# dbekaert/RAiDER

Hardware: AMD Instinct MI355X
Metric: LOS rays/sec (wet+hydro slant delay) through ERA5 cube; achieved HBM GB/s (higher is better)
Workload: dtype f64; 1 GPU; configs[2]: Raytracing LOS, 4000x4000 scene (16.0M rays), one slice at ht=0, per-pixel ECEF look vectors, synthetic ERA5-sized 300x300x80 f32 cube, zref=max(z)-1, MAX_SEGMENT_LENGTH=1000; rays_per_gpu=16000000, cube=300x300x80, levels_K=76, parallelism=single GPU, ranks=1, world_size_seen_by_backend=1, devices_visible=1, ranks_per_device=1, distinct_devices=1

## Files before the change

### include/raider_hip.h

```cpp
#ifndef RAIDER_HIP_H
#define RAIDER_HIP_H

#include <stdint.h>

#ifdef __cplusplus
extern "C" {
#endif

#define RDR_OK 0
#define RDR_ERR_INVALID (-1)
#define RDR_ERR_HIP (-2)
#define RDR_ERR_NODEVICE (-3)
#define RDR_ERR_ALL_NAN (-4)
#define RDR_ERR_NO_LEVELS (-5)
#define RDR_ERR_NAN_LENGTH (-6)
#define RDR_ERR_OOM (-7)

#define RDR_F32 0
#define RDR_F64 1
#define RDR_I16 2
#define RDR_BYTESWAPPED 0x100
#define RDR_HOST 0
#define RDR_DEVICE 1

// ... 57 lines not shown
int rdr_clock_sample_end(rdr_ctx* ctx, double* ghz);
int rdr_ray_kernel_attributes(rdr_ctx* ctx, const rdr_cube* cube, int which, int32_t* vgprs, int32_t* static_lds, int32_t* dynamic_lds,
                              int32_t* scratch, int32_t* max_threads);
int64_t rdr_generic_ray_count(rdr_ctx* ctx);
int64_t rdr_skipped_wave_count(rdr_ctx* ctx);

int rdr_cube_create(rdr_ctx* ctx, const double* ys, int64_t ny, const double* xs, int64_t nx,
                    const double* zs, int64_t nz, const void* wet, const void* hydro, int dtype,
                    int64_t sy, int64_t sx, int64_t sz, int loc, rdr_cube** out);
void rdr_cube_destroy(rdr_cube* cube);
int rdr_cube_has_nan(const rdr_cube* cube);
int rdr_cube_shape(const rdr_cube* cube, int64_t* ny, int64_t* nx, int64_t* nz, int* dtype);
int rdr_cube_axes(const rdr_cube* cube, double* ys, double* xs, double* zs);
#define RDR_PROJ_LONLAT 0
#define RDR_PROJ_LCC 1
#define RDR_PROJ_STERE 2
int rdr_cube_set_projection(rdr_cube* cube, int kind, const double* params, int nparams);
int rdr_cube_view(rdr_ctx* ctx, const rdr_cube* cube, int kind, const double* params, int nparams, rdr_cube** out);
int rdr_project_points(rdr_ctx* ctx, const rdr_cube* cube, const double* lat, const double* lon, int64_t n, double* y, double* x, int loc);
int rdr_transform_tm(rdr_ctx* ctx, const double* params, int nparams, int direction, const double* in_a, const double* in_b, int64_t n,
                     double* out_a, double* out_b, int loc);
int rdr_transform_cone(rdr_ctx* ctx, int kind, const double* params, int nparams, int direction, const double* in_a, const double* in_b,
                       int64_t n, double* out_a, double* out_b, int loc);
#define RDR_GRID_TM 3
int rdr_grid_geodetic(rdr_ctx* ctx, int grid_kind, const double* params, int nparams, const double* xpts, int64_t nx, const double* ypts,
                      int64_t ny, double* lat, double* lon, int loc);
int rdr_cube_blend(rdr_ctx* ctx, const rdr_cube* a, double w1, const rdr_cube* b, double w2, rdr_cube** out);
int rdr_inverse_time_weights(rdr_ctx* ctx, const double* az, int64_t n, const double* dates, int32_t nd, double window_s,
                             double regularizer, double* weights, int loc);
int rdr_cube_blend_weighted(rdr_ctx* ctx, const rdr_cube* const* cubes, int32_t nd, const double* weights, int loc, rdr_cube** out);
int rdr_cube_blend_azimuth_time(rdr_ctx* ctx, const rdr_cube* const* pointwise, const rdr_cube* const* total, int32_t nd, const double* lat2d,
                                const double* lon2d, int loc, const double* sv_t, const double* sv_pos, const double* sv_vel, int64_t nsv,
                                const double* dates_s, double window_s, double reg, int64_t offset_us, rdr_cube** out_pointwise,
                                rdr_cube** out_total, double* time_grid, int32_t* flags);

int rdr_delays_to_phase(rdr_ctx* ctx, const void* wet, const void* hydro, int64_t n, int dtype, double wavelength,
                        void* wet_out, void* hydro_out, int loc);

int rdr_cube_read(rdr_ctx* ctx, const rdr_cube* cube, void* wet, void* hydro);

int rdr_interp3(rdr_ctx* ctx, const rdr_cube* cube, const double* pts, int64_t n, double* wet,
                double* hydro, int loc);
int rdr_interp3_project(rdr_ctx* ctx, const rdr_cube* cube, const double* y, const double* x, const double* z, int64_t n, int proj_mode,
                        const double* proj, double inc0, double* wet, double* hydro, int loc);
int rdr_cube_point_index(rdr_ctx* ctx, rdr_cube* cube, int mode);
int64_t rdr_cube_point_index_bytes(const rdr_cube* cube);
int rdr_build_cube(rdr_ctx* ctx, const rdr_cube* cube, const double* xpts, int64_t nx, const double* ypts,
                   int64_t ny, const double* zpts, int64_t nz, double* wet, double* hydro, int loc);
int rdr_build_cube_grid(rdr_ctx* ctx, const rdr_cube* cube, int grid_kind, const double* params, int nparams, const double* xpts, int64_t nx,
                        const double* ypts, int64_t ny, const double* zpts, int64_t nz, double* wet, double* hydro, int loc);
int rdr_last_nan_output(rdr_ctx* ctx);
int rdr_build_cube_to_cube(rdr_ctx* ctx, const rdr_cube* cube, const double* xpts, int64_t nx, const double* ypts, int64_t ny,
                           const double* zpts, int64_t nz, int loc, rdr_cube** out);
int rdr_build_cube_grid_to_cube(rdr_ctx* ctx, const rdr_cube* cube, int grid_kind, const double* params, int nparams, const double* xpts,
                                int64_t nx, const double* ypts, int64_t ny, const double* zpts, int64_t nz, int loc, rdr_cube** out);
int rdr_interp3_blend(rdr_ctx* ctx, const rdr_cube* a, double w1, const rdr_cube* b, double w2, const double* y, const double* x, const double* z,
                      int64_t n, double* wet, double* hydro, int loc);
int rdr_interp3_blend_cube(rdr_ctx* ctx, const rdr_cube* a, double w1, const rdr_cube* b, double w2, const double* y, const double* x, const double* z,
                           int64_t n, double* wet, double* hydro, int loc);
int rdr_point_delays(rdr_ctx* ctx, const rdr_cube* cube, const double* xpts, int64_t nx, const double* ypts, int64_t ny, const double* zpts,
                     int64_t nz, const double* y, const double* x, const double* z, int64_t n, int proj_mode, const double* proj, double inc0,
                     double* wet, double* hydro, int32_t* cube_has_nan);
int rdr_point_delays_grid(rdr_ctx* ctx, const rdr_cube* cube, int grid_kind, const double* params, int nparams, const double* xpts, int64_t nx,
                          const double* ypts, int64_t ny, const double* zpts, int64_t nz, const double* y, const double* x, const double* z, int64_t n,
                          int proj_mode, const double* proj, double inc0, double* wet, double* hydro, int32_t* cube_has_nan);
int rdr_interp3_project_epochs(rdr_ctx* ctx, const rdr_cube* const* cubes, int32_t ncubes, const double* y, const double* x, const double* z,
                               int64_t n, int proj_mode, const double* proj, int64_t proj_stride, double inc0, double* wet, double* hydro, int loc);
int rdr_point_delays_epochs(rdr_ctx* ctx, const rdr_cube* const* cubes, int32_t ncubes, int grid_kind, const double* params, int nparams,
                            const double* xpts, int64_t nx, const double* ypts, int64_t ny, const double* zpts, int64_t nz, const double* y,
                            const double* x, const double* z, int64_t n, int proj_mode, const double* proj, int64_t proj_stride, double inc0,
                            double* wet, double* hydro, int32_t* cube_has_nan);
int64_t rdr_point_upload_bytes(const rdr_ctx* ctx);
int rdr_project_cosinc(rdr_ctx* ctx, double* wet, double* hydro, const double* inc, int64_t n, int loc);
int rdr_project_divide(rdr_ctx* ctx, double* wet, double* hydro, const double* divisor, int64_t n, int loc);

int rdr_ray_levels(const rdr_cube* cube, double ht, double zref, int32_t* K, double* lo, double* hi, int32_t* kz);
int rdr_ray_prepass(rdr_ctx* ctx, const rdr_cube* cube, const rdr_rays* rays, double ht, double zref,
                    double* maxlen, int32_t* flags);
int rdr_nparts(const double* maxlen, int32_t K, double max_seg, int32_t* nparts);
int rdr_ray_prepass_device(rdr_ctx* ctx, const rdr_cube* cube, const rdr_rays* rays, double ht, double zref, double* partition);
int rdr_ray_march_device(rdr_ctx* ctx, const rdr_cube* cube, const rdr_rays* rays, double ht, double zref, double max_seg,
                         const double* partition, double* wet, double* hydro);

int rdr_ray_march(rdr_ctx* ctx, const rdr_cube* cube, const rdr_rays* rays, double ht, double zref,
                  const int32_t* nparts, int32_t flags, double* wet, double* hydro);
int rdr_raytrace(rdr_ctx* ctx, const rdr_cube* cube, const rdr_rays* rays, double ht, double zref,
                 double max_seg, double* wet, double* hydro, int32_t* nparts_out, int32_t* flags_out);

int rdr_raytrace_slices(rdr_ctx* ctx, const rdr_cube* cube, const rdr_rays* rays, const double* hts, int32_t nslices,
                        int32_t los_per_slice, double zref, double max_seg, double* wet, double* hydro, int32_t* K_out,
                        int32_t* nparts_out, int32_t ld, int32_t* flags_out);

int rdr_raytrace_slices_to_cube(rdr_ctx* ctx, const rdr_cube* cube, const rdr_rays* rays, const double* hts, int32_t nslices,
                                int32_t los_per_slice, double zref, double max_seg, int32_t* K_out, int32_t* nparts_out, int32_t ld,
                                int32_t* flags_out, rdr_cube** out);

int rdr_raytrace_slices_epochs(rdr_ctx* ctx, const rdr_cube* const* cubes, int32_t ncubes, const rdr_rays* rays, const double* hts,
                               int32_t nslices, int32_t los_per_slice, double zref, double max_seg, double* wet, double* hydro,
                               int32_t* K_out, int32_t* nparts_out, int32_t ld, int32_t* flags_out);

int rdr_raytrace_slices_epochs_to_cubes(rdr_ctx* ctx, const rdr_cube* const* cubes, int32_t ncubes, const rdr_rays* rays,
                                        const double* hts, int32_t nslices, int32_t los_per_slice, double zref, double max_seg,
                                        int32_t* K_out, int32_t* nparts_out, int32_t ld, int32_t* flags_out, rdr_cube** out);

int rdr_raytrace_epochs(rdr_ctx* ctx, const rdr_cube* const* cubes, int32_t ncubes, const rdr_rays* rays, double ht, double zref,
                        double max_seg, double* wet, double* hydro, int32_t* nparts_out, int32_t* flags_out);

int rdr_top_of_atmosphere(rdr_ctx* ctx, const double* xyz, const double* los, int64_t n, double toaheight,
                          const double* factor, double* pos, int loc);
int rdr_build_ray(rdr_ctx* ctx, const double* model_zs, int64_t nz, double ht, const double* xyz,
                  const double* los, int64_t n, double zref, int32_t* K, double* lengths, double* low,
                  double* high, int loc);

int rdr_lla2ecef(rdr_ctx* ctx, const double* lat, const double* lon, const double* h, int64_t n, double* xyz, int loc);
int rdr_ecef2lla(rdr_ctx* ctx, const double* xyz, int64_t n, double* lon, double* lat, double* h, int loc);
int rdr_look_vectors(rdr_ctx* ctx, const rdr_rays* rays, double ht, double* los);

int rdr_ecmwf_model_levels(rdr_ctx* ctx, const float* z_surf, const float* lnsp, const float* t, const float* q, const float* lats,
                           const double* a, const double* b, int32_t nlev, int64_t ny, int64_t nx, double R_d,
                           double* p_out, double* zs_out, int loc);

int rdr_pressure_level_state(rdr_ctx* ctx, const double* height, int height_kind, const double* p, int p_ndim, const double* t,
                             const double* hum, const double* lats, int lat_ndim, int64_t nlev, int64_t ny, int64_t nx,
                             int top_first, int rows_descending, int cols_descending, double* zs_out, double* p_out,
                             double* t_out, double* hum_out, int loc, int out_loc);

int rdr_cubes_from_model_levels(rdr_ctx* ctx, const double* ys, int64_t ny, const double* xs, int64_t nx, const double* zs3,
                                const double* p, const double* t, const double* hum, int humidity_type, int64_t nlev,
                                const double* new_z, int64_t nz, double k1, double k2, double k3, double zmin, int loc,
                                rdr_cube** pointwise, rdr_cube** total, float* t_out, float* p_out, float* e_out);

int rdr_orbit_look_vectors(rdr_ctx* ctx, const double* sv_t, const double* sv_pos, const double* sv_vel, int64_t nsv,
                           const double* xyz, int64_t n, double threshold, int maxiter, double* los, double* aztime,
                           double* srange, int loc);

int rdr_interp_nd(rdr_ctx* ctx, int32_t ndim, const double* const* axes, const int64_t* axis_len,
                  const double* values, const double* interp_points, int64_t n, int has_fill,
                  double fill_value, double* out, int loc);
int rdr_interp_along_axis(rdr_ctx* ctx, const double* points, const double* values, int64_t ncol, int64_t m,
                          const double* interp_points, int64_t mq, int has_fill, double fill_value,
                          double* out, int loc);
int64_t rdr_make_points_count(double max_len, double step);
int rdr_make_points(rdr_ctx* ctx, double max_len, const double* sp, const double* slv, int64_t nrays,
                    double step, double* out, int loc);

int rdr_raster_sample(rdr_ctx* ctx, const void* raster, int dtype, int64_t height, int64_t width, const double* gt6, const double* x,
                      const double* y, int64_t n, int method, int has_nodata, double nodata, double* out, int loc);
int rdr_raster_bounds(rdr_ctx* ctx, const void* a, const void* b, int dtype, int64_t n, int has_nodata, double nodata, double* out6, int loc);

int rdr_tiff_lzw_decode(rdr_ctx* ctx, const void* src, int64_t src_bytes, const int64_t* seg_offset, const int64_t* seg_bytes, int64_t nseg,
                        const int64_t* seg_out_bytes, void* out, int64_t out_stride, int32_t* status, int loc);
int rdr_tiff_assemble(rdr_ctx* ctx, const void* segs, int64_t seg_stride, int64_t height, int64_t width, int64_t tile_h, int64_t tile_w,
                      int predictor, int swap, int sample_bytes, int planar, int bands, int band, void* out, int loc);
int rdr_tiff_predict(rdr_ctx* ctx, const void* in, int sample_bytes, int64_t height, int64_t width, void* out, int loc);

int64_t rdr_deflate_bound(int64_t n);
int rdr_deflate_encode(rdr_ctx* ctx, const void* src, int64_t src_bytes, const int64_t* seg_offset, const int64_t* seg_bytes, int64_t nseg,
                       void* out, int64_t out_capacity, int64_t* out_offset, int loc);
int rdr_h5_chunks(rdr_ctx* ctx, const void* array, int elem_bytes, int ndim, const int64_t* shape, const int64_t* chunk, const void* fill,
                  int shuffle, void* out, int loc);

#ifdef __cplusplus
}
#endif
#endif
```

### raider_amd/_lib.py

```python
import ctypes as C
import os
import threading
from pathlib import Path

import numpy as np

_HERE = Path(__file__).resolve().parent
LIB_PATH = Path(os.environ.get('RAIDER_HIP_LIB', _HERE / 'libraider_hip.so'))

RDR_OK = 0
RDR_ERR_INVALID, RDR_ERR_HIP, RDR_ERR_NODEVICE, RDR_ERR_ALL_NAN, RDR_ERR_NO_LEVELS, RDR_ERR_NAN_LENGTH, RDR_ERR_OOM = -1, -2, -3, -4, -5, -6, -7
RDR_F32, RDR_F64, RDR_I16 = 0, 1, 2
RASTER_NEAREST, RASTER_LINEAR = 0, 1
RDR_BYTESWAPPED = 0x100
RDR_HOST, RDR_DEVICE = 0, 1
ORIGIN_GRID, ORIGIN_LLH, ORIGIN_XYZ = 0, 1, 2
RDR_PROJ_LCC, RDR_PROJ_STERE, RDR_GRID_TM = 1, 2, 3
LOS_VEC, LOS_INC_HD, LOS_INC_HD_SCALAR, LOS_ZENITH = 0, 1, 2, 3
ORBIT_LDS_MAX_SV = 320
FLAG_ANY_NAN, FLAG_ANY_FINITE, FLAG_FIRST_NOT_BELOW, FLAG_LAST_NOT_ABOVE, FLAG_DIVERGED, FLAG_BAD_HEIGHT, FLAG_NAN_OUTPUT = 1, 2, 4, 8, 16, 32, 64

c_dp = C.POINTER(C.c_double)
c_ip = C.POINTER(C.c_int32)
c_lp = C.POINTER(C.c_int64)
# ... 19 lines not shown


_lib = None
_lock = threading.Lock()

_VP = C.c_void_p
SYMBOLS = [
    ('rdr_version', C.c_int, []),
    ('rdr_source_hash', C.c_char_p, []),
    ('rdr_create', C.c_int, [C.c_int, C.POINTER(_VP)]),
    ('rdr_destroy', None, [_VP]),
    ('rdr_last_error', C.c_char_p, [_VP]),
    ('rdr_set_stream', C.c_int, [_VP, _VP]),
    ('rdr_forget_stream', C.c_int, [_VP, _VP]),
    ('rdr_synchronize', C.c_int, [_VP]),
    ('rdr_device_info', C.c_int, [_VP, C.c_char_p, C.c_int, C.POINTER(C.c_int), c_lp]),
    ('rdr_set_profiling', C.c_int, [_VP, C.c_int]),
    ('rdr_host_alloc', C.c_int, [C.c_int64, C.POINTER(_VP)]),
    ('rdr_host_free', C.c_int, [_VP]),
    ('rdr_set_workspace_limit', C.c_int, [_VP, C.c_int64]),
    ('rdr_set_side_capacity', C.c_int, [_VP, C.c_int64]),
    ('rdr_trim', C.c_int, [_VP, C.c_int64, c_lp]),
    ('rdr_generic_ray_count', C.c_int64, [_VP]),
    ('rdr_skipped_wave_count', C.c_int64, [_VP]),
    ('rdr_profile_get', C.c_int, [_VP, C.c_int, C.POINTER(C.c_int), C.POINTER(C.c_float)]),
    ('rdr_clock_sample_begin', C.c_int, [_VP, C.c_double]),
    ('rdr_clock_sample_end', C.c_int, [_VP, c_dp]),
    ('rdr_ray_kernel_attributes', C.c_int, [_VP, _VP, C.c_int, c_ip, c_ip, c_ip, c_ip, c_ip]),
    ('rdr_cube_create', C.c_int, [_VP, _VP, C.c_int64, _VP, C.c_int64, _VP, C.c_int64, _VP, _VP, C.c_int,
                                  C.c_int64, C.c_int64, C.c_int64, C.c_int, C.POINTER(_VP)]),
    ('rdr_cube_destroy', None, [_VP]),
    ('rdr_cube_has_nan', C.c_int, [_VP]),
    ('rdr_cube_shape', C.c_int, [_VP, c_lp, c_lp, c_lp, C.POINTER(C.c_int)]),
    ('rdr_cube_axes', C.c_int, [_VP, _VP, _VP, _VP]),
    ('rdr_cube_set_projection', C.c_int, [_VP, C.c_int, _VP, C.c_int]),
    ('rdr_cube_view', C.c_int, [_VP, _VP, C.c_int, _VP, C.c_int, C.POINTER(_VP)]),
    ('rdr_project_points', C.c_int, [_VP, _VP, _VP, _VP, C.c_int64, _VP, _VP, C.c_int]),
    ('rdr_transform_tm', C.c_int, [_VP, _VP, C.c_int, C.c_int, _VP, _VP, C.c_int64, _VP, _VP, C.c_int]),
    ('rdr_transform_cone', C.c_int, [_VP, C.c_int, _VP, C.c_int, C.c_int, _VP, _VP, C.c_int64, _VP, _VP, C.c_int]),
    ('rdr_grid_geodetic', C.c_int, [_VP, C.c_int, _VP, C.c_int, _VP, C.c_int64, _VP, C.c_int64, _VP, _VP, C.c_int]),
    ('rdr_cube_blend', C.c_int, [_VP, _VP, C.c_double, _VP, C.c_double, C.POINTER(_VP)]),
    ('rdr_cube_read', C.c_int, [_VP, _VP, _VP, _VP]),
    ('rdr_cube_point_index', C.c_int, [_VP, _VP, C.c_int]),
    ('rdr_cube_point_index_bytes', C.c_int64, [_VP]),
    ('rdr_interp3', C.c_int, [_VP, _VP, _VP, C.c_int64, _VP, _VP, C.c_int]),
    ('rdr_interp3_project', C.c_int, [_VP, _VP, _VP, _VP, _VP, C.c_int64, C.c_int, _VP, C.c_double, _VP, _VP, C.c_int]),
    ('rdr_interp3_blend', C.c_int, [_VP, _VP, C.c_double, _VP, C.c_double, _VP, _VP, _VP, C.c_int64, _VP, _VP, C.c_int]),
    ('rdr_interp3_blend_cube', C.c_int, [_VP, _VP, C.c_double, _VP, C.c_double, _VP, _VP, _VP, C.c_int64, _VP, _VP, C.c_int]),
    ('rdr_build_cube', C.c_int, [_VP, _VP, _VP, C.c_int64, _VP, C.c_int64, _VP, C.c_int64, _VP, _VP, C.c_int]),
    ('rdr_build_cube_to_cube', C.c_int, [_VP, _VP, _VP, C.c_int64, _VP, C.c_int64, _VP, C.c_int64, C.c_int, C.POINTER(_VP)]),
    ('rdr_build_cube_grid', C.c_int, [_VP, _VP, C.c_int, _VP, C.c_int, _VP, C.c_int64, _VP, C.c_int64, _VP, C.c_int64, _VP, _VP, C.c_int]),
    ('rdr_build_cube_grid_to_cube', C.c_int, [_VP, _VP, C.c_int, _VP, C.c_int, _VP, C.c_int64, _VP, C.c_int64, _VP, C.c_int64, C.c_int, C.POINTER(_VP)]),
    ('rdr_last_nan_output', C.c_int, [_VP]),
    ('rdr_point_delays', C.c_int, [_VP, _VP, _VP, C.c_int64, _VP, C.c_int64, _VP, C.c_int64, _VP, _VP, _VP, C.c_int64, C.c_int, _VP, C.c_double, _VP, _VP,
                                   c_ip]),
    ('rdr_point_delays_grid', C.c_int, [_VP, _VP, C.c_int, _VP, C.c_int, _VP, C.c_int64, _VP, C.c_int64, _VP, C.c_int64, _VP, _VP, _VP, C.c_int64, C.c_int,
                                        _VP, C.c_double, _VP, _VP, c_ip]),
    ('rdr_interp3_project_epochs', C.c_int, [_VP, C.POINTER(_VP), C.c_int32, _VP, _VP, _VP, C.c_int64, C.c_int, _VP, C.c_int64, C.c_double, _VP, _VP, C.c_int]),
    ('rdr_point_delays_epochs', C.c_int, [_VP, C.POINTER(_VP), C.c_int32, C.c_int, _VP, C.c_int, _VP, C.c_int64, _VP, C.c_int64, _VP, C.c_int64, _VP, _VP, _VP,
                                          C.c_int64, C.c_int, _VP, C.c_int64, C.c_double, _VP, _VP, c_ip]),
    ('rdr_point_upload_bytes', C.c_int64, [_VP]),
    ('rdr_project_cosinc', C.c_int, [_VP, _VP, _VP, _VP, C.c_int64, C.c_int]),
    ('rdr_project_divide', C.c_int, [_VP, _VP, _VP, _VP, C.c_int64, C.c_int]),
    ('rdr_ray_levels', C.c_int, [_VP, C.c_double, C.c_double, c_ip, _VP, _VP, _VP]),
    ('rdr_ray_prepass', C.c_int, [_VP, _VP, C.POINTER(RdrRays), C.c_double, C.c_double, _VP, c_ip]),
    ('rdr_nparts', C.c_int, [_VP, C.c_int32, C.c_double, _VP]),
    ('rdr_ray_march', C.c_int, [_VP, _VP, C.POINTER(RdrRays), C.c_double, C.c_double, _VP, C.c_int32, _VP, _VP]),
    ('rdr_raytrace', C.c_int, [_VP, _VP, C.POINTER(RdrRays), C.c_double, C.c_double, C.c_double, _VP, _VP, _VP, c_ip]),
    ('rdr_raytrace_slices', C.c_int, [_VP, _VP, C.POINTER(RdrRays), _VP, C.c_int32, C.c_int32, C.c_double, C.c_double, _VP, _VP, _VP, _VP, C.c_int32, _VP]),
    ('rdr_raytrace_slices_to_cube', C.c_int, [_VP, _VP, C.POINTER(RdrRays), _VP, C.c_int32, C.c_int32, C.c_double, C.c_double, _VP, _VP, C.c_int32, _VP,
                                              C.POINTER(_VP)]),
    ('rdr_raytrace_slices_epochs', C.c_int, [_VP, C.POINTER(_VP), C.c_int32, C.POINTER(RdrRays), _VP, C.c_int32, C.c_int32, C.c_double, C.c_double,
                                             _VP, _VP, _VP, _VP, C.c_int32, _VP]),
    ('rdr_raytrace_slices_epochs_to_cubes', C.c_int, [_VP, C.POINTER(_VP), C.c_int32, C.POINTER(RdrRays), _VP, C.c_int32, C.c_int32, C.c_double,
                                                      C.c_double, _VP, _VP, C.c_int32, _VP, C.POINTER(_VP)]),
    ('rdr_raytrace_epochs', C.c_int, [_VP, C.POINTER(_VP), C.c_int32, C.POINTER(RdrRays), C.c_double, C.c_double, C.c_double, _VP, _VP, _VP, c_ip]),
    ('rdr_top_of_atmosphere', C.c_int, [_VP, _VP, _VP, C.c_int64, C.c_double, _VP, _VP, C.c_int]),
    ('rdr_build_ray', C.c_int, [_VP, _VP, C.c_int64, C.c_double, _VP, _VP, C.c_int64, C.c_double, c_ip, _VP, _VP, _VP, C.c_int]),
    ('rdr_lla2ecef', C.c_int, [_VP, _VP, _VP, _VP, C.c_int64, _VP, C.c_int]),
    ('rdr_ecef2lla', C.c_int, [_VP, _VP, C.c_int64, _VP, _VP, _VP, C.c_int]),
    ('rdr_look_vectors', C.c_int, [_VP, C.POINTER(RdrRays), C.c_double, _VP]),
    ('rdr_ray_prepass_device', C.c_int, [_VP, _VP, _VP, C.c_double, C.c_double, _VP]),
    ('rdr_ray_march_device', C.c_int, [_VP, _VP, _VP, C.c_double, C.c_double, C.c_double, _VP, _VP, _VP]),
    ('rdr_inverse_time_weights', C.c_int, [_VP, _VP, C.c_int64, _VP, C.c_int32, C.c_double, C.c_double, _VP, C.c_int]),
    ('rdr_cube_blend_weighted', C.c_int, [_VP, C.POINTER(_VP), C.c_int32, _VP, C.c_int, C.POINTER(_VP)]),
    ('rdr_cube_blend_azimuth_time', C.c_int, [_VP, C.POINTER(_VP), C.POINTER(_VP), C.c_int32, _VP, _VP, C.c_int, _VP, _VP, _VP, C.c_int64, _VP, C.c_double,
                                              C.c_double, C.c_int64, C.POINTER(_VP), C.POINTER(_VP), _VP, c_ip]),
    ('rdr_delays_to_phase', C.c_int, [_VP, _VP, _VP, C.c_int64, C.c_int, C.c_double, _VP, _VP, C.c_int]),
    ('rdr_ecmwf_model_levels', C.c_int, [_VP, _VP, _VP, _VP, _VP, _VP, _VP, _VP, C.c_int32, C.c_int64, C.c_int64, C.c_double, _VP, _VP, C.c_int]),
    ('rdr_pressure_level_state', C.c_int, [_VP, _VP, C.c_int, _VP, C.c_int, _VP, _VP, _VP, C.c_int, C.c_int64, C.c_int64, C.c_int64, C.c_int, C.c_int,
                                           C.c_int, _VP, _VP, _VP, _VP, C.c_int, C.c_int]),
    ('rdr_cubes_from_model_levels', C.c_int, [_VP, _VP, C.c_int64, _VP, C.c_int64, _VP, _VP, _VP, _VP, C.c_int, C.c_int64, _VP, C.c_int64,
                                              C.c_double, C.c_double, C.c_double, C.c_double, C.c_int, C.POINTER(_VP), C.POINTER(_VP), _VP, _VP, _VP]),
    ('rdr_orbit_look_vectors', C.c_int, [_VP, _VP, _VP, _VP, C.c_int64, _VP, C.c_int64, C.c_double, C.c_int, _VP, _VP, _VP, C.c_int]),
    ('rdr_interp_nd', C.c_int, [_VP, C.c_int32, C.POINTER(_VP), c_lp, _VP, _VP, C.c_int64, C.c_int, C.c_double, _VP, C.c_int]),
    ('rdr_interp_along_axis', C.c_int, [_VP, _VP, _VP, C.c_int64, C.c_int64, _VP, C.c_int64, C.c_int, C.c_double, _VP, C.c_int]),
    ('rdr_make_points_count', C.c_int64, [C.c_double, C.c_double]),
    ('rdr_make_points', C.c_int, [_VP, C.c_double, _VP, _VP, C.c_int64, C.c_double, _VP, C.c_int]),
    ('rdr_raster_sample', C.c_int, [_VP, _VP, C.c_int, C.c_int64, C.c_int64, _VP, _VP, _VP, C.c_int64, C.c_int, C.c_int, C.c_double, _VP, C.c_int]),
    ('rdr_raster_bounds', C.c_int, [_VP, _VP, _VP, C.c_int, C.c_int64, C.c_int, C.c_double, _VP, C.c_int]),
    ('rdr_tiff_lzw_decode', C.c_int, [_VP, _VP, C.c_int64, _VP, _VP, C.c_int64, _VP, _VP, C.c_int64, _VP, C.c_int]),
    ('rdr_tiff_assemble', C.c_int, [_VP, _VP, C.c_int64, C.c_int64, C.c_int64, C.c_int64, C.c_int64, C.c_int, C.c_int, C.c_int, C.c_int, C.c_int, C.c_int,
                                    _VP, C.c_int]),
    ('rdr_tiff_predict', C.c_int, [_VP, _VP, C.c_int, C.c_int64, C.c_int64, _VP, C.c_int]),
    ('rdr_deflate_bound', C.c_int64, [C.c_int64]),
    ('rdr_deflate_encode', C.c_int, [_VP, _VP, C.c_int64, _VP, _VP, C.c_int64, _VP, C.c_int64, _VP, C.c_int]),
    ('rdr_h5_chunks', C.c_int, [_VP, _VP, C.c_int, C.c_int, _VP, _VP, _VP, C.c_int, _VP, C.c_int]),
]


def _preload_hip_runtime():
    import importlib.util
    import sys
    choice = os.environ.get('RAIDER_HIP_RUNTIME', '')
    if choice == 'system' or 'torch' in sys.modules:
        return
    if choice:
        C.CDLL(choice, mode=C.RTLD_GLOBAL)
        return
    try:
        spec = importlib.util.find_spec('torch')
    except (ImportError, ValueError):
        spec = None
    if spec and spec.submodule_search_locations:
        cand = Path(list(spec.submodule_search_locations)[0]) / 'lib' / 'libamdhip64.so'
        if cand.exists():
            C.CDLL(str(cand), mode=C.RTLD_GLOBAL)


def source_files():
    return sorted(f for f in (_HERE / 'csrc').glob('*') if f.suffix in ('.h', '.hip')) + [_HERE.parent / 'include' / 'raider_hip.h']


def source_hash():
    import hashlib
    h = hashlib.sha256()
    for f in source_files():
        h.update(f.name.encode()); h.update(f.read_bytes())
    return h.hexdigest()[:16]


def binary_source_hash(path=None):
    path = Path(path or LIB_PATH)
    if not path.exists():
        return None
    if _lib is not None and path == LIB_PATH:
        return _lib.rdr_source_hash().decode()
    data = path.read_bytes()
    k = data.find(b'rdr-source-hash:')
    if k < 0:
        return None
    return data[k + 16:k + 32].decode(errors='replace')


def load():
    global _lib
    with _lock:
        if _lib is not None:
            return _lib
        if not LIB_PATH.exists():
            raise RuntimeError(
                f'raider_amd: HIP library {LIB_PATH} is missing - build it with '
                f'`python -c "import __graft_entry__ as g; g.build()"` (hipcc --offload-arch=gfx950). '
                'There is no CPU fallback.')
        _preload_hip_runtime()
        lib = C.CDLL(str(LIB_PATH))
# ... 157 lines not shown
```

### raider_amd/csrc/epoch_kernels.h

```cpp
#pragma once
#include "raider_kernels.h"
#include "cube_kernels.h"

namespace rdr {

constexpr int EPOCHS_MAX = 4;

template <typename T2, int E, bool PR>
struct EpochWaves {
    static constexpr int value = PR ? (sizeof(T2) == 8 ? (E <= 2 ? 3 : 2) : (E <= 2 ? 2 : 1)) : ((sizeof(T2) == 8 && E <= 2) ? 3 : 2);
};

template <typename T2, int E, int GRID, bool PR>
__global__ __launch_bounds__(BLOCK) __attribute__((amdgpu_waves_per_eu(EpochWaves<T2, E, PR>::value, EpochWaves<T2, E, PR>::value)))
void march_epochs_kernel(CubeView<T2> c_in, EpochCubes<T2, E> ev, RayParams P, int64_t estride) {
    static_assert(!PR || GRID == 0 || GRID == 1, "per-ray heights: REGULAR or run-time flags");
    constexpr bool REGULAR = GRID == 1;
    CubeView<T2> c = c_in;
    if (REGULAR) { c.exact_y = 1; c.exact_x = 1; c.small = 1; }
    if (GRID == 2) { c.exact_y = 0; c.exact_x = 0; c.uni_y = 1; c.uni_x = 1; c.small = 1; }
    extern __shared__ __attribute__((aligned(16))) unsigned char smem_raw[];
    const RaySmem m = carve_smem(smem_raw, c.ny, c.nx, c.nz, c.exact_y, c.exact_x);
    fill_axes(c, m);
    int K = 0, slice = -1;
    double poison = 0.0;
    bool clamp_lo = false, clamp_hi = false;
    TileWalk walk(P.tile_count, P.tile_ctr, m.K + 2);
    int64_t lt;
    while (walk.next(P.tile_count, lt)) {
        const int64_t tg = P.tile_begin + lt;
        const int sl = (int)(tg / P.tiles_per_slice);
        const int64_t t = tg - (int64_t)sl * P.tiles_per_slice;
        if (sl != slice) {
            slice = sl;
            K = fill_levels(c.nz, m, P.hts ? P.hts[sl] : P.ht, P.zref);
            const SlicePartition part = fill_partition<!PR>(P, m, c.nz, sl, K);
            poison = part.poison; clamp_lo = part.clamp_lo; clamp_hi = part.clamp_hi;
        }
        int tl = threadIdx.x;
        asm volatile("" : "+v"(tl));
        int64_t i; bool active;
        tile_ray(P, t, tl, i, active);
        const double* w = P.ws + (lt * BLOCK + tl);
        const int64_t ns = P.nslots;
        const double scale_rec = w[(int64_t)WS_SCALE * ns];
        const bool mine = !active || scale_rec != 0.0;
        int k0 = 0; double lo_first = K > 0 ? m.lo[0] : 0.0;
        if constexpr (PR) k0 = (active && mine) ? first_level(m.ax.ez, c.nz, m.lo, m.hi, m.kz, K, P.ht_ray[i], lo_first) : K;
        double acc_w[E], acc_h[E];
#pragma unroll
        for (int e = 0; e < E; ++e) { acc_w[e] = 0.0; acc_h[e] = 0.0; }
        RayPoly q;
        double xc[PX];
        load_ray_record(w, ns, q, xc);
        const double scale = scale_rec;
        const double u0r = w[(int64_t)WS_U0 * ns], u1r = w[(int64_t)WS_U1 * ns];
        const unsigned long long live = __builtin_amdgcn_ballot_w64(active && mine);
        auto run = [&](auto nochk) {
            constexpr bool NC = decltype(nochk)::value;
            if constexpr (PR) march_ray_height_levels<T2, E, NC>(c, ev, m, q, xc, u0r, u1r, K, k0, lo_first, clamp_lo, clamp_hi, acc_w, acc_h);
            else march_slice_levels<T2, E, NC>(c, ev, m, q, xc, u0r, u1r, K, clamp_lo, clamp_hi, live, acc_w, acc_h);
        };
        bool lane_safe = false;
        if (REGULAR) lane_safe = lane_nocheck(u0r, u1r, active, mine, q, xc, c.ny, c.nx);
        if (REGULAR && __all(lane_safe)) run(std::integral_constant<bool, true>{});
        else run(std::integral_constant<bool, false>{});
        if (active && scale_rec != 0.0) {
            const int64_t o = (int64_t)sl * P.n + i;
#pragma unroll
            for (int e = 0; e < E; ++e) {
                const double aw = acc_w[e] * scale, ah = acc_h[e] * scale;
                P.wet[e * estride + o] = aw + poison; P.hyd[e * estride + o] = ah + poison;
            }
        }
    }
}

template <typename T2, int E>
__global__ __launch_bounds__(256) void interp_points_epochs_kernel(CubeView<T2> c, EpochCubes<T2, E> ev, PointQuery Q, int64_t pstride, int64_t n, int64_t estride,
                                                                   double* __restrict__ wet, double* __restrict__ hyd, int axes_in_lds) {
    PlainCorners<T2> src[E];
#pragma unroll
    for (int e = 0; e < E; ++e) src[e].v = ev.v[e];
    gather_points<E>(c, src, Q, pstride, n, estride, wet, hyd, axes_in_lds);
}

}
```

### raider_amd/csrc/raider_hip.hip

```cpp
#include <hip/hip_runtime.h>

#include <algorithm>
#include <atomic>
#include <cmath>
#include <cstdio>
#include <cstdlib>
#include <cstring>
#include <functional>
#include <mutex>
#include <string>
#include <utility>
#include <vector>

#include "../../include/raider_hip.h"
#include "raider_kernels.h"

using namespace rdr;

static thread_local std::string g_err;

struct DevBuf {
    void* p = nullptr;
    size_t cap = 0;
};

constexpr int MAX_SLICES = 512;

enum { SLOT_IN0 = 0, SLOT_IN1, SLOT_IN2, SLOT_IN3, SLOT_IN4, SLOT_IN5, SLOT_IN6, SLOT_OUT0, SLOT_OUT1, SLOT_OUT2, SLOT_AUX,
       SLOT_PT0, SLOT_PT1, SLOT_PT2, SLOT_PT3, SLOT_PT4, SLOT_PT5, SLOT_TMPCUBE, SLOT_TMPAXES,
       SLOT_DEFL,
       NSLOT };

struct rdr_ctx {
    int device = 0;
    hipStream_t own_stream = nullptr;
    hipStream_t copy_stream = nullptr;
    hipStream_t down_stream = nullptr;
    hipStream_t stream = nullptr;
    int num_cus = 256;
    size_t lds_max = 64u << 10;
    size_t total_mem = 0;
    std::string name;
    bool profiling = false;
    std::vector<std::pair<hipEvent_t, hipEvent_t>> evs[4];
    size_t ev_used[4] = {0, 0, 0, 0};
    DevBuf slot[NSLOT];
    unsigned long long* d_maxlen = nullptr;
    int* d_flags = nullptr;
    int* d_nparts = nullptr;
    int* d_nslow = nullptr;
    int* d_tilectr = nullptr;
    struct PoolEntry { void* p; size_t bytes; std::vector<hipEvent_t> evs; };
    std::vector<PoolEntry> cube_pool;
    std::vector<hipStream_t> ext_streams;
    bool ext_overflow = false;
    size_t cube_pool_bytes = 0, cube_pool_limit = (size_t)4 << 30;
    DevBuf ws;
    DevBuf side;
    int64_t side_cap = 0;
    int* d_sidectr = nullptr;
    int* h_word = nullptr;
    struct PinSlot { void* p = nullptr; size_t cap = 0; hipEvent_t ev = nullptr; bool used = false; };
    static constexpr int PIN_SLOTS = 16;
    static constexpr size_t PIN_MAX = (size_t)1 << 20;
    PinSlot pin[PIN_SLOTS];
    int pin_next = 0;
    hipEvent_t staged_ev = nullptr;
    static constexpr int NAN_SLOTS = 256;
    int* nan_words = nullptr;
    const struct rdr_cube* nan_owner[NAN_SLOTS] = {};
    int nan_next = 0;
    int64_t side_forced = -1;
    int64_t last_nskip = 0;
    int64_t last_nslow = 0;
    int wall_khz = 0;
    int64_t point_upload_bytes = 0;
    int last_nan_output = -1;
    size_t ws_limit = (size_t)48 << 30;
    struct { const void* cube = nullptr; const void* vals = nullptr; LccParams proj = {0, 0, 0, 0, 0, 0, 0, 0}; int64_t n = -1; double ht = 0, zref = 0; const void* a = nullptr; const void* b = nullptr; const void* c = nullptr; const void* d = nullptr; int K = 0; bool valid = false; } wsig;
    std::string err;
};

struct rdr_cube {
    rdr_ctx* ctx = nullptr;
    int64_t ny = 0, nx = 0, nz = 0;
    int dtype = RDR_F32;
    void* d_vals = nullptr;
    double* d_axes = nullptr;
    std::vector<double> ys, xs, zs;
    int uni[3] = {0, 0, 0};
    int exact[2] = {0, 0};
    double inv_d[3] = {0, 0, 0};
    LccParams proj = {0, 0, 0, 0, 0, 0, 0, 0};
    mutable void* d_quad = nullptr;
    mutable size_t quad_bytes = 0;
    mutable int quad_nblk = 0;
    mutable int big_point_calls = 0;
    mutable std::mutex quad_mutex;
    mutable bool has_nan = false;
    mutable hipEvent_t ready_ev = nullptr;
    hipStream_t ready_stream = nullptr;
    mutable int nan_slot = -1;
    size_t alloc_bytes = 0;
    const rdr_cube* base = nullptr;
    mutable int views = 0;
    mutable bool doomed = false;
    mutable std::atomic<bool> foreign{false};
    mutable std::vector<hipStream_t> used_streams;
    mutable std::atomic<hipStream_t> last_stream{nullptr};
};
static std::recursive_mutex g_view_mutex;
static inline const rdr_cube* root(const rdr_cube* q) { return q->base ? q->base : q; }
static inline void note_use(const rdr_ctx* c, const rdr_cube* q) {
    if (!c || !q) return;
    const rdr_cube* r = root(q);
    if (r->ctx != c) r->foreign.store(true, std::memory_order_relaxed);
    if (r->last_stream.load(std::memory_order_relaxed) != c->stream) {
        std::lock_guard<std::recursive_mutex> guard(g_view_mutex);
        if (std::find(r->used_streams.begin(), r->used_streams.end(), c->stream) == r->used_streams.end()) r->used_streams.push_back(c->stream);
        r->last_stream.store(c->stream, std::memory_order_relaxed);
    }
    if (r->ready_ev && r->ready_stream != c->stream) { (void)hipStreamWaitEvent(c->stream, r->ready_ev, 0); (void)hipGetLastError(); }
}
static void cube_resolve_nan(const rdr_cube* r) {
    std::lock_guard<std::recursive_mutex> guard(g_view_mutex);
    if (r->nan_slot < 0) return;
    rdr_ctx* c = r->ctx;
    if (r->ready_ev) (void)hipEventSynchronize(r->ready_ev);
    r->has_nan = c->nan_words[r->nan_slot] != 0;
    c->nan_owner[r->nan_slot] = nullptr;
    r->nan_slot = -1;
}


static int fail(rdr_ctx* ctx, int code, const std::string& msg) {
    g_err = msg;
    if (ctx) ctx->err = msg;
    return code;
}

#define HIPCHECK(ctx, expr)                                                                         \
    do {                                                                                            \
// ... 144 lines not shown
    hipLaunchKernelGGL(kern, g, b, sm, s, std::forward<Args>(args)...);
    return hipGetLastError();
}

#include "cube_kernels.h"
#include "producer_kernels.h"
#include "orbit_kernels.h"
#include "aztime_kernels.h"
#include "native_kernels.h"
#include "proj_kernels.h"
#include "epoch_kernels.h"
#include "raster_kernels.h"
#include "tiff_kernels.h"
#include "deflate_kernels.h"


int rdr_version(void) { return 102; }

#ifndef RDR_SOURCE_HASH
#define RDR_SOURCE_HASH "unknown"
#endif
static const char k_source_hash[] = "rdr-source-hash:" RDR_SOURCE_HASH;
const char* rdr_source_hash(void) { return k_source_hash + 16; }

const char* rdr_last_error(rdr_ctx* ctx) { return (ctx && !ctx->err.empty()) ? ctx->err.c_str() : g_err.c_str(); }

int rdr_create(int device, rdr_ctx** out) {
    if (!out) return fail(nullptr, RDR_ERR_INVALID, "rdr_create: out is NULL");
    *out = nullptr;
    int count = 0;
    hipError_t e = hipGetDeviceCount(&count);
    if (e != hipSuccess || count <= 0)
        return fail(nullptr, RDR_ERR_NODEVICE, std::string("rdr_create: no HIP device available (") +
                    (e != hipSuccess ? hipGetErrorString(e) : "device count 0") + "); raider_amd has no CPU fallback");
    if (device < 0) { if (hipGetDevice(&device) != hipSuccess) device = 0; }
    if (device >= count) return fail(nullptr, RDR_ERR_INVALID, "rdr_create: device index out of range");
    rdr_ctx* c = new rdr_ctx();
    c->device = device;
    const int rc = [&]() -> int {
        HIPCHECK(nullptr, hipSetDevice(device));
        hipDeviceProp_t prop;
        HIPCHECK(nullptr, hipGetDeviceProperties(&prop, device));
        c->num_cus = prop.multiProcessorCount;
        c->total_mem = prop.totalGlobalMem;
        c->lds_max = std::max<size_t>(prop.sharedMemPerBlock, prop.maxSharedMemoryPerMultiProcessor);
        c->name = prop.name;
        if (c->name.empty()) c->name = std::string("AMD ") + prop.gcnArchName;
        HIPCHECK(nullptr, hipStreamCreateWithFlags(&c->own_stream, hipStreamNonBlocking));
        HIPCHECK(nullptr, hipStreamCreateWithFlags(&c->copy_stream, hipStreamNonBlocking));
        HIPCHECK(nullptr, hipStreamCreateWithFlags(&c->down_stream, hipStreamNonBlocking));
        c->stream = c->own_stream;
        HIPCHECK(nullptr, hipMalloc((void**)&c->d_maxlen, (size_t)MAX_SLICES * MAX_LEVELS * sizeof(unsigned long long)));
        HIPCHECK(nullptr, hipMalloc((void**)&c->d_flags, (MAX_SLICES + 4) * sizeof(int)));
        HIPCHECK(nullptr, hipMalloc((void**)&c->d_nparts, MAX_LEVELS * sizeof(int)));
        HIPCHECK(nullptr, hipMalloc((void**)&c->d_nslow, 2 * sizeof(int)));
        HIPCHECK(nullptr, hipMalloc((void**)&c->d_tilectr, 32 * sizeof(int)));
        HIPCHECK(nullptr, hipMalloc((void**)&c->d_sidectr, sizeof(int)));
        HIPCHECK(nullptr, hipMemset(c->d_sidectr, 0, sizeof(int)));
        HIPCHECK(nullptr, hipHostMalloc((void**)&c->h_word, 16 * sizeof(int), hipHostMallocDefault));
        HIPCHECK(nullptr, hipHostMalloc((void**)&c->nan_words, rdr_ctx::NAN_SLOTS * sizeof(int), hipHostMallocDefault));
        HIPCHECK(nullptr, hipMemset(c->d_nslow, 0, 2 * sizeof(int)));
        return RDR_OK;
    }();
    if (rc) { rdr_destroy(c); return rc; }
    if (const char* e = std::getenv("RAIDER_HIP_WORKSPACE_BYTES")) c->ws_limit = (size_t)std::strtoull(e, nullptr, 10);
    if (const char* e = std::getenv("RAIDER_HIP_CUBE_POOL_BYTES")) c->cube_pool_limit = (size_t)std::strtoull(e, nullptr, 10);
    *out = c;
    return RDR_OK;
}

void rdr_destroy(rdr_ctx* c) {
    if (!c) return;
    (void)hipSetDevice(c->device);
    if (c->stream) (void)hipStreamSynchronize(c->stream);
    for (auto& b : c->slot) if (b.p) (void)hipFree(b.p);
    for (auto& e : c->cube_pool) { for (auto ev : e.evs) (void)hipEventDestroy(ev); (void)hipFree(e.p); }
    if (c->d_maxlen) (void)hipFree(c->d_maxlen);
    if (c->d_flags) (void)hipFree(c->d_flags);
    if (c->d_nparts) (void)hipFree(c->d_nparts);
    if (c->d_nslow) (void)hipFree(c->d_nslow);
    if (c->d_tilectr) (void)hipFree(c->d_tilectr);
    if (c->ws.p) (void)hipFree(c->ws.p);
    if (c->side.p) (void)hipFree(c->side.p);
    if (c->d_sidectr) (void)hipFree(c->d_sidectr);
    if (c->h_word) (void)hipHostFree(c->h_word);
    if (c->nan_words) (void)hipHostFree(c->nan_words);
    for (auto& ps : c->pin) { if (ps.ev) (void)hipEventDestroy(ps.ev); if (ps.p) (void)hipHostFree(ps.p); }
    if (c->staged_ev) (void)hipEventDestroy(c->staged_ev);
    for (auto& v : c->evs) for (auto& pr : v) { (void)hipEventDestroy(pr.first); (void)hipEventDestroy(pr.second); }
    if (c->own_stream) (void)hipStreamDestroy(c->own_stream);
    if (c->copy_stream) (void)hipStreamDestroy(c->copy_stream);
    if (c->down_stream) (void)hipStreamDestroy(c->down_stream);
    delete c;
}

int rdr_set_stream(rdr_ctx* c, void* s) {
    if (!c) return fail(nullptr, RDR_ERR_INVALID, "ctx is NULL");
    const hipStream_t before = c->stream;
    const hipStream_t want = (s == (void*)(intptr_t)-1) ? c->own_stream : (hipStream_t)s;
    if (want != before) {
        hipEvent_t ev = nullptr;
        if (hipEventCreateWithFlags(&ev, hipEventDisableTiming) == hipSuccess) {
            if (hipEventRecord(ev, before) == hipSuccess) (void)hipStreamWaitEvent(want, ev, 0);
            (void)hipEventDestroy(ev);
        }
        (void)hipGetLastError();
    }
    if (s == (void*)(intptr_t)-1) c->stream = c->own_stream;
    else {
        c->stream = (hipStream_t)s;
        std::lock_guard<std::recursive_mutex> guard(g_view_mutex);
        if (std::find(c->ext_streams.begin(), c->ext_streams.end(), c->stream) == c->ext_streams.end()) {
            if (c->ext_streams.size() < 8) c->ext_streams.push_back(c->stream); else c->ext_overflow = true;
        }
    }
    return RDR_OK;
}

int rdr_forget_stream(rdr_ctx* c, void* s) {
    if (!c) return fail(nullptr, RDR_ERR_INVALID, "ctx is NULL");
    const hipStream_t st = (hipStream_t)s;
    if (c->stream == st && st != c->own_stream) {
        HIPCHECK(c, hipStreamSynchronize(st));
        c->stream = c->own_stream;
    }
    std::lock_guard<std::recursive_mutex> guard(g_view_mutex);
    c->ext_streams.erase(std::remove(c->ext_streams.begin(), c->ext_streams.end(), st), c->ext_streams.end());
    if (c->ext_streams.size() < 8) c->ext_overflow = false;
    return RDR_OK;
}

int rdr_synchronize(rdr_ctx* c) {
    if (!c) return fail(nullptr, RDR_ERR_INVALID, "ctx is NULL");
    HIPCHECK(c, hipStreamSynchronize(c->stream));
    return RDR_OK;
}

int rdr_device_info(rdr_ctx* c, char* name, int name_len, int* cus, int64_t* mem) {
    if (!c) return fail(nullptr, RDR_ERR_INVALID, "ctx is NULL");
    if (name && name_len > 0) { std::strncpy(name, c->name.c_str(), name_len - 1); name[name_len - 1] = 0; }
    if (cus) *cus = c->num_cus;
    if (mem) *mem = (int64_t)c->total_mem;
    return RDR_OK;
}

int rdr_host_alloc(int64_t bytes, void** out) {
    if (!out || bytes <= 0) return fail(nullptr, RDR_ERR_INVALID, "rdr_host_alloc: bad argument");
    void* p = nullptr;
    const hipError_t e = hipHostMalloc(&p, (size_t)bytes, hipHostMallocDefault);
    if (e != hipSuccess) return fail(nullptr, RDR_ERR_HIP, std::string("hipHostMalloc: ") + hipGetErrorString(e));
    *out = p;
    return RDR_OK;
}

int rdr_host_free(void* p) {
    if (!p) return RDR_OK;
    const hipError_t e = hipHostFree(p);
    if (e != hipSuccess) return fail(nullptr, RDR_ERR_HIP, std::string("hipHostFree: ") + hipGetErrorString(e));
    return RDR_OK;
}

int rdr_set_workspace_limit(rdr_ctx* c, int64_t bytes) {
    if (!c || bytes < (int64_t)1 << 20) return fail(c, RDR_ERR_INVALID, "rdr_set_workspace_limit: need at least 1 MiB");
    c->ws_limit = (size_t)bytes;
    c->wsig.valid = false;
    return RDR_OK;
}

static void pool_drain(rdr_ctx* c) {
    std::lock_guard<std::recursive_mutex> guard(g_view_mutex);
    while (!c->cube_pool.empty()) {
        rdr_ctx::PoolEntry e = c->cube_pool.front();
        c->cube_pool.erase(c->cube_pool.begin());
        c->cube_pool_bytes -= e.bytes;
        for (auto ev : e.evs) { (void)hipEventSynchronize(ev); (void)hipEventDestroy(ev); }
        (void)hipFree(e.p);
    }
    (void)hipGetLastError();
}

int rdr_trim(rdr_ctx* c, int64_t keep_bytes, int64_t* released) {
    if (!c || keep_bytes < 0) return fail(c, RDR_ERR_INVALID, "rdr_trim: NULL context or a negative size");
    HIPCHECK(c, hipSetDevice(c->device));
    HIPCHECK(c, hipStreamSynchronize(c->down_stream));
    HIPCHECK(c, hipStreamSynchronize(c->copy_stream));
    HIPCHECK(c, hipStreamSynchronize(c->stream));
    if (c->stream != c->own_stream) HIPCHECK(c, hipStreamSynchronize(c->own_stream));
    const size_t keep = (size_t)keep_bytes;
    size_t freed = 0;
    auto drop = [&](DevBuf& b) { if (b.p && b.cap > keep) { if (hipFree(b.p) == hipSuccess) freed += b.cap; b.p = nullptr; b.cap = 0; } };
    for (auto& b : c->slot) drop(b);
    if ((c->ws.p && c->ws.cap > keep) || (c->side.p && c->side.cap > keep)) c->wsig.valid = false;
    drop(c->ws);
    if (c->side.p && c->side.cap > keep) { drop(c->side); c->side_cap = 0; }
    std::lock_guard<std::recursive_mutex> guard(g_view_mutex);
    while (!c->cube_pool.empty() && c->cube_pool_bytes > keep) {
        rdr_ctx::PoolEntry e = c->cube_pool.front();
        c->cube_pool.erase(c->cube_pool.begin());
        c->cube_pool_bytes -= e.bytes;
        for (auto ev : e.evs) { (void)hipEventSynchronize(ev); (void)hipEventDestroy(ev); }
        if (hipFree(e.p) == hipSuccess) freed += e.bytes;
    }
    (void)hipGetLastError();
    if (released) *released = (int64_t)freed;
    return RDR_OK;
}

int rdr_set_side_capacity(rdr_ctx* c, int64_t columns) {
    if (!c) return fail(nullptr, RDR_ERR_INVALID, "ctx is NULL");
    c->side_forced = columns < 0 ? -1 : columns;
    c->wsig.valid = false;
    return RDR_OK;
}

int64_t rdr_generic_ray_count(rdr_ctx* c) { return c ? c->last_nslow : -1; }
int64_t rdr_skipped_wave_count(rdr_ctx* c) { return c ? c->last_nskip : -1; }

int rdr_set_profiling(rdr_ctx* c, int on) {
    if (!c) return fail(nullptr, RDR_ERR_INVALID, "ctx is NULL");
    c->profiling = on != 0;
    for (auto& u : c->ev_used) u = 0;
    return RDR_OK;
}

__global__ void clock_sample_kernel(long long wall_ticks, long long* out) {
    if (threadIdx.x != 0) return;
    const long long c0 = clock64(), w0 = wall_clock64();
    while (wall_clock64() - w0 < wall_ticks) __builtin_amdgcn_s_sleep(127);
    const long long c1 = clock64(), w1 = wall_clock64();
    out[0] = c1 - c0; out[1] = w1 - w0;
}

int rdr_clock_sample_begin(rdr_ctx* c, double ms) {
    if (!c || !(ms > 0) || ms > 60000.0) return fail(c, RDR_ERR_INVALID, "rdr_clock_sample_begin: NULL context or a duration outside (0, 60000] ms");
    HIPCHECK(c, hipSetDevice(c->device));
    int khz = 0;
    HIPCHECK(c, hipDeviceGetAttribute(&khz, hipDeviceAttributeWallClockRate, c->device));
    if (khz <= 0) return fail(c, RDR_ERR_HIP, "rdr_clock_sample_begin: the device reports no wall-clock rate");
    long long* out = reinterpret_cast<long long*>(c->h_word + 4);
    out[0] = 0; out[1] = 0;
    c->wall_khz = khz;
    hipLaunchKernelGGL(clock_sample_kernel, dim3(1), dim3(64), 0, c->copy_stream, (long long)(ms * khz), out);
    HIPCHECK(c, hipGetLastError());
    return RDR_OK;
}

int rdr_clock_sample_end(rdr_ctx* c, double* ghz) {
    if (!c || !ghz) return fail(c, RDR_ERR_INVALID, "rdr_clock_sample_end: NULL argument");
    HIPCHECK(c, hipSetDevice(c->device));
    HIPCHECK(c, hipStreamSynchronize(c->copy_stream));
    const long long* out = reinterpret_cast<const long long*>(c->h_word + 4);
    if (out[1] <= 0 || c->wall_khz <= 0) return fail(c, RDR_ERR_INVALID, "rdr_clock_sample_end: no sample was started on this context");
    *ghz = (double)out[0] / ((double)out[1] / (c->wall_khz * 1e3)) / 1e9;
    return RDR_OK;
}

int rdr_profile_get(rdr_ctx* c, int which, int* count, float* total_ms) {
    if (!c || which < 0 || which > 3 || !count || !total_ms) return fail(c, RDR_ERR_INVALID, "rdr_profile_get: bad argument");
    float tot = 0;
    for (size_t i = 0; i < c->ev_used[which]; ++i) {
        float ms = 0;
        HIPCHECK(c, hipEventSynchronize(c->evs[which][i].second));
        HIPCHECK(c, hipEventElapsedTime(&ms, c->evs[which][i].first, c->evs[which][i].second));
        tot += ms;
    }
    *count = (int)c->ev_used[which];
    *total_ms = tot;
    return RDR_OK;
}

static int axis_check(const double* g, int64_t n, int* flip) {
    if (n < 2) return -1;
    bool asc = true, desc = true;
    for (int64_t i = 1; i < n; ++i) {
        if (!(g[i] > g[i - 1])) asc = false;
        if (!(g[i] < g[i - 1])) desc = false;
    }
// ... 1259 lines not shown
    c->wsig.cube = q; c->wsig.vals = q->d_vals; c->wsig.proj = q->proj; c->wsig.n = r->n; c->wsig.ht = ht; c->wsig.zref = zref; c->wsig.K = K; c->wsig.valid = valid;
    c->wsig.a = r->origin_mode == RDR_ORIGIN_GRID ? (const void*)r->xpts : (r->origin_mode == RDR_ORIGIN_XYZ ? (const void*)r->xyz : (const void*)r->lat);
    c->wsig.b = r->origin_mode == RDR_ORIGIN_GRID ? (const void*)r->ypts : (const void*)r->lon;
    c->wsig.c = r->los_mode == RDR_LOS_VEC ? (const void*)r->los : (const void*)r->inc;
    c->wsig.d = (const void*)r->hts;
}

static bool wsig_match(rdr_ctx* c, const rdr_cube* q, const rdr_rays* r, double ht, double zref, int K) {
    if (!c->wsig.valid || c->wsig.cube != q || c->wsig.vals != q->d_vals || std::memcmp(&c->wsig.proj, &q->proj, sizeof(LccParams)) != 0 || c->wsig.n != r->n || c->wsig.ht != ht || c->wsig.zref != zref || c->wsig.K != K) return false;
    if (r->loc != RDR_DEVICE) return false;
    const void* a = r->origin_mode == RDR_ORIGIN_GRID ? (const void*)r->xpts : (r->origin_mode == RDR_ORIGIN_XYZ ? (const void*)r->xyz : (const void*)r->lat);
    const void* b = r->origin_mode == RDR_ORIGIN_GRID ? (const void*)r->ypts : (const void*)r->lon;
    const void* cc = r->los_mode == RDR_LOS_VEC ? (const void*)r->los : (const void*)r->inc;
    return a == c->wsig.a && b == c->wsig.b && cc == c->wsig.c && (const void*)r->hts == c->wsig.d;
}

static bool pass1_skip_on() {
    static const int on = []() { const char* e = std::getenv("RAIDER_HIP_PASS1_SKIP"); return e ? std::atoi(e) : 1; }();
    return on != 0;
}

template <typename T2>
static auto crossings_fn(bool lcc, int om, bool per_ray) -> void (*)(CubeView<T2>, RayParams, LccParams) {
#define RDR_X(LCC_, OM_) (per_ray ? crossings_kernel<T2, false, LCC_, OM_, true> : crossings_kernel<T2, false, LCC_, OM_, false>)
#define RDR_X_OM(LCC_) (om == 1 ? RDR_X(LCC_, 1) : om == 2 ? RDR_X(LCC_, 2) : RDR_X(LCC_, 0))
    return lcc ? RDR_X_OM(true) : RDR_X_OM(false);
#undef RDR_X_OM
#undef RDR_X
}

template <typename T2>
static auto march_fn(int grid, bool per_ray) -> void (*)(CubeView<T2>, RayParams, LccParams) {
    if (per_ray) return grid == 1 ? march_kernel<T2, false, 1, true> : march_kernel<T2, false, 0, true>;
    return grid == 1 ? march_kernel<T2, false, 1> : grid == 2 ? march_kernel<T2, false, 2> : march_kernel<T2, false, 0>;
}

template <typename T2, int E>
static auto march_epochs_fn(int grid, bool per_ray) -> void (*)(CubeView<T2>, EpochCubes<T2, E>, RayParams, int64_t) {
    if (per_ray) return grid == 1 ? march_epochs_kernel<T2, E, 1, true> : march_epochs_kernel<T2, E, 0, true>;
    return grid == 1 ? march_epochs_kernel<T2, E, 1, false> : grid == 2 ? march_epochs_kernel<T2, E, 2, false> : march_epochs_kernel<T2, E, 0, false>;
}

static int launch_crossings(rdr_ctx* c, const rdr_cube* q, RayParams P, int64_t tb, int64_t tc, int64_t nslots_total = 0, bool reset_nslow = true) {
    P.tile_begin = tb; P.tile_count = tc; P.nslots = nslots_total > 0 ? nslots_total : tc * BLOCK;
    const bool skippable = pass1_skip_on() && q->proj.kind != 1 && !P.ht_ray && P.maxlen_bits != nullptr &&
                           ray_lds_total(q) + skip_smem_bytes(q->nz) <= c->lds_max;
    P.skip_levels = skippable ? 1 : 0;
    const int g = ray_grid(c, tc, 8);
    if (ray_lds_total(q) > c->lds_max)
        return fail(c, RDR_ERR_INVALID, "ray tracing: the cube's non-uniform horizontal axes and level tables need " + std::to_string(ray_lds_total(q)) +
                    " B of LDS per workgroup, the device offers " + std::to_string(c->lds_max) + " (resample the cube to uniform axes or crop it)");
    if (reset_nslow) {
        HIPCHECK(c, hipMemsetAsync(c->d_nslow, 0, 2 * sizeof(int), c->stream));
        HIPCHECK(c, hipMemsetAsync(c->d_sidectr, 0, sizeof(int), c->stream));
    }
    HIPCHECK(c, hipMemsetAsync(c->d_tilectr, 0, 16 * sizeof(int), c->stream));
    P.tile_ctr = c->d_tilectr;
    const size_t sm = ray_smem(q);
    hipError_t e = hipSuccess;
    {
        KTimer t(c, 0);
        const size_t sm_light = sm + (skippable ? skip_smem_bytes(q->nz) : 0);
        const bool lcc = q->proj.kind == 1;
        const int om = P.origin_mode != RDR_ORIGIN_GRID ? 0 : (P.los_mode == RDR_LOS_VEC ? 1 : 2);
        const dim3 G(g), B(BLOCK);
        e = q->dtype == RDR_F32 ? launch_lds(crossings_fn<float2>(lcc, om, P.ht_ray != nullptr), G, B, sm_light, c->stream, make_view<float2>(q), P, q->proj)
                                : launch_lds(crossings_fn<double2>(lcc, om, P.ht_ray != nullptr), G, B, sm_light, c->stream, make_view<double2>(q), P, q->proj);
    }
    if (e != hipSuccess) return fail(c, RDR_ERR_HIP, std::string("crossings_kernel launch: ") + hipGetErrorString(e));
    P.tile_ctr = c->d_tilectr + 8;
    if (q->dtype == RDR_F32) e = launch_lds(crossings_kernel<float2, true>, dim3(g), dim3(BLOCK), sm, c->stream, make_view<float2>(q), P, q->proj);
    else e = launch_lds(crossings_kernel<double2, true>, dim3(g), dim3(BLOCK), sm, c->stream, make_view<double2>(q), P, q->proj);
    if (e != hipSuccess) return fail(c, RDR_ERR_HIP, std::string("crossings_kernel launch: ") + hipGetErrorString(e));
    return RDR_OK;
}

static int march_grid(const rdr_cube* q, bool per_ray) {
    const bool small = make_view<float2>(q).small && (q->dtype == RDR_F32 || make_view<double2>(q).small);
    if (!small) return 0;
    if (q->exact[0] && q->exact[1]) return 1;
    return (!per_ray && !q->exact[0] && !q->exact[1] && q->uni[0] && q->uni[1]) ? 2 : 0;
}

static int launch_march_generic(rdr_ctx* c, const rdr_cube* q, RayParams P, dim3 G, dim3 B, size_t sm, bool zero_ctr) {
    if (zero_ctr) HIPCHECK(c, hipMemsetAsync(c->d_tilectr + 24, 0, 8 * sizeof(int), c->stream));
    P.tile_ctr = c->d_tilectr + 24;
    hipError_t e;
    if (q->dtype == RDR_F32) e = launch_lds(march_kernel<float2, true>, G, B, sm, c->stream, make_view<float2>(q), P, q->proj);
    else e = launch_lds(march_kernel<double2, true>, G, B, sm, c->stream, make_view<double2>(q), P, q->proj);
    if (e != hipSuccess) return fail(c, RDR_ERR_HIP, std::string("march_kernel launch: ") + hipGetErrorString(e));
    return RDR_OK;
}

static int launch_march(rdr_ctx* c, const rdr_cube* q, RayParams P, int64_t tb, int64_t tc, int64_t nslots_total = 0) {
    P.tile_begin = tb; P.tile_count = tc; P.nslots = nslots_total > 0 ? nslots_total : tc * BLOCK;
    static const int stage_f64 = []() { const char* e = std::getenv("RAIDER_HIP_F64_STAGE"); return e ? std::atoi(e) : 1; }();
    P.stage_f64 = stage_f64;
    const int g = ray_grid(c, tc, 8);
    HIPCHECK(c, hipMemsetAsync(c->d_tilectr + 16, 0, 16 * sizeof(int), c->stream));
    P.tile_ctr = c->d_tilectr + 16;
    const size_t sm = ray_smem(q);
    const dim3 G(g), B(BLOCK);
    hipError_t e = hipSuccess;
    {
        KTimer t(c, 1);
        const bool per_ray = P.ht_ray != nullptr;
        const int grid = march_grid(q, per_ray);
        e = q->dtype == RDR_F32 ? launch_lds(march_fn<float2>(grid, per_ray), G, B, sm, c->stream, make_view<float2>(q), P, q->proj)
                                : launch_lds(march_fn<double2>(grid, per_ray), G, B, sm, c->stream, make_view<double2>(q), P, q->proj);
    }
    if (e != hipSuccess) return fail(c, RDR_ERR_HIP, std::string("march_kernel launch: ") + hipGetErrorString(e));
    return launch_march_generic(c, q, P, G, B, sm, false);
}

static int epochs_max() {
    const char* e = std::getenv("RAIDER_HIP_EPOCHS_MAX");
    const int v = e ? std::atoi(e) : EPOCHS_MAX;
    return v >= 4 ? 4 : v >= 2 ? 2 : 1;
}

static int epoch_group(int dtype, bool per_ray, int left, int emax) {
    if (per_ray && dtype == RDR_F64) {
        const char* env = std::getenv("RAIDER_HIP_EPOCHS_PR_F64_MAX");
        emax = std::min(emax, env ? std::atoi(env) : 2);
    }
    return (left >= 4 && emax >= 4) ? 4 : (left >= 2 && emax >= 2) ? 2 : 1;
}

template <typename T2, int E>
static hipError_t launch_stacked(rdr_ctx* c, const rdr_cube* const* qs, int grid, const RayParams& P, int64_t estride, dim3 G, dim3 B, size_t sm) {
    EpochCubes<T2, E> ev;
    for (int j = 0; j < E; ++j) ev.v[j] = (const T2*)qs[j]->d_vals;
    return launch_lds(march_epochs_fn<T2, E>(grid, P.ht_ray != nullptr), G, B, sm, c->stream, make_view<T2>(qs[0]), ev, P, estride);
}

static int launch_march_epochs(rdr_ctx* c, const rdr_cube* const* qs, int D, RayParams P, int64_t tb, int64_t tc, int64_t estride) {
    const rdr_cube* q = qs[0];
    const int emax = epochs_max();
    const bool per_ray = P.ht_ray != nullptr;
    const int grid = march_grid(q, per_ray);
    const int g = ray_grid(c, tc, 8);
    const size_t sm = ray_smem(q);
    const dim3 G(g), B(BLOCK);
    for (int e = 0; e < D;) {
        const int ge = epoch_group(q->dtype, per_ray, D - e, emax);
        RayParams Pe = P;
        Pe.wet = P.wet + (int64_t)e * estride; Pe.hyd = P.hyd + (int64_t)e * estride;
        if (ge == 1) {
            const int rc = launch_march(c, qs[e], Pe, tb, tc); if (rc) return rc;
            ++e;
            continue;
        }
        Pe.tile_begin = tb; Pe.tile_count = tc; Pe.nslots = tc * BLOCK;
        HIPCHECK(c, hipMemsetAsync(c->d_tilectr + 16, 0, 8 * sizeof(int), c->stream));
        Pe.tile_ctr = c->d_tilectr + 16;
        hipError_t err = hipSuccess;
        {
            KTimer t(c, 1);
            if (q->dtype == RDR_F32) err = ge == 4 ? launch_stacked<float2, 4>(c, qs + e, grid, Pe, estride, G, B, sm) : launch_stacked<float2, 2>(c, qs + e, grid, Pe, estride, G, B, sm);
            else err = ge == 4 ? launch_stacked<double2, 4>(c, qs + e, grid, Pe, estride, G, B, sm) : launch_stacked<double2, 2>(c, qs + e, grid, Pe, estride, G, B, sm);
        }
        if (err != hipSuccess) return fail(c, RDR_ERR_HIP, std::string("march_epochs_kernel launch: ") + hipGetErrorString(err));
        for (int j = 0; j < ge; ++j) {
            RayParams Pj = Pe;
            Pj.wet = Pe.wet + (int64_t)j * estride; Pj.hyd = Pe.hyd + (int64_t)j * estride;
            const int rc = launch_march_generic(c, qs[e + j], Pj, G, B, sm, true); if (rc) return rc;
        }
        e += ge;
    }
    return RDR_OK;
}

int rdr_ray_kernel_attributes(rdr_ctx* c, const rdr_cube* q, int which, int32_t* vgprs, int32_t* static_lds, int32_t* dynamic_lds,
                              int32_t* scratch, int32_t* max_threads) {
    if (!c || !q || which < 0 || which > 7) return fail(c, RDR_ERR_INVALID, "rdr_ray_kernel_attributes: bad argument");
    const void* fn = nullptr;
    const bool lcc = q->proj.kind == 1;
    const bool pr = which == 2 || which == 3 || which >= 6;
    const int grid = march_grid(q, pr);
    const bool f32 = q->dtype == RDR_F32;
    if (which >= 4) {
        if ((which & 1) != 0) fn = f32 ? (const void*)march_epochs_fn<float2, 4>(grid, pr) : (const void*)march_epochs_fn<double2, 4>(grid, pr);
        else fn = f32 ? (const void*)march_epochs_fn<float2, 2>(grid, pr) : (const void*)march_epochs_fn<double2, 2>(grid, pr);
    } else if ((which & 1) == 0) fn = f32 ? (const void*)crossings_fn<float2>(lcc, 1, pr) : (const void*)crossings_fn<double2>(lcc, 1, pr);
    else fn = f32 ? (const void*)march_fn<float2>(grid, pr) : (const void*)march_fn<double2>(grid, pr);
    hipFuncAttributes a;
    HIPCHECK(c, hipFuncGetAttributes(&a, fn));
    if (vgprs) *vgprs = a.numRegs;
    if (static_lds) *static_lds = (int32_t)a.sharedSizeBytes;
    if (dynamic_lds) *dynamic_lds = (int32_t)ray_smem(q);
    if (scratch) *scratch = (int32_t)a.localSizeBytes;
    if (max_threads) *max_threads = a.maxThreadsPerBlock;
    return RDR_OK;
}

static int ray_passes(rdr_ctx* c, const rdr_cube* q, const RayParams& P, int K, int64_t per, int64_t nslices, int64_t fit, int64_t max_group,
                      bool reduce, const std::function<int(const RayParams&, int64_t, int64_t)>& march = nullptr,
                      const std::function<int(int64_t, int64_t)>& after_group = nullptr) {
    const auto pass2 = [&](const RayParams& Pm, int64_t tb, int64_t tc) { return march ? march(Pm, tb, tc) : launch_march(c, q, Pm, tb, tc); };
    if (per <= fit) {
        const int64_t g = std::min<int64_t>(max_group, std::max<int64_t>(1, fit / per));
        for (int64_t s0 = 0; s0 < nslices; s0 += g) {
            const int64_t ns = std::min<int64_t>(g, nslices - s0);
            RayParams Pg = P;
            if (!reduce) Pg.maxlen_bits = nullptr;
            int rc = ws_reserve(c, ns * per, K, Pg); if (rc) return rc;
            rc = launch_crossings(c, q, Pg, s0 * per, ns * per); if (rc) return rc;
            Pg.maxlen_bits = P.maxlen_bits;
            rc = pass2(Pg, s0 * per, ns * per); if (rc) return rc;
            if (after_group) { rc = after_group(s0, ns); if (rc) return rc; }
        }
        return RDR_OK;
    }
    for (int64_t s = 0; s < nslices; ++s) {
        int rc;
        if (reduce) {
            RayParams Ps = P;
            Ps.ws = nullptr;
            rc = launch_crossings(c, q, Ps, s * per, per); if (rc) return rc;
        }
        RayParams Pw = P;
        rc = ws_reserve(c, fit, K, Pw); if (rc) return rc;
        for (int64_t tb = 0; tb < per; tb += fit) {
            const int64_t tc = std::min<int64_t>(fit, per - tb);
            RayParams Pc = Pw;
            Pc.maxlen_bits = nullptr;
            rc = launch_crossings(c, q, Pc, s * per + tb, tc); if (rc) return rc;
            Pc.maxlen_bits = P.maxlen_bits;
            rc = pass2(Pc, s * per + tb, tc); if (rc) return rc;
        }
    }
    return RDR_OK;
}

static int raytrace_pipelined(rdr_ctx* c, const rdr_cube* q, const rdr_rays* r, RayParams P, int K, double* d_los, double* d_hts, double* dw, double* dh,
                              double* wet, double* hydro) {
    const int64_t tile_rows = P.ntiles / P.tiles_x;
    const int nchunk = (int)std::min<int64_t>(8, tile_rows);
    int rc = ws_reserve(c, P.ntiles, K, P); if (rc) return rc;
    double* const ws = P.ws;
    const int64_t nslots_total = P.ntiles * BLOCK;
    if (d_los) P.los = d_los;
    if (d_hts) P.ht_ray = d_hts;
    std::vector<hipEvent_t> ev(2 * nchunk, nullptr);
    auto range = [&](int k, int64_t& tb, int64_t& tc, int64_t& r0, int64_t& cnt) {
        const int64_t t0 = tile_rows * k / nchunk, t1 = tile_rows * (k + 1) / nchunk;
        tb = t0 * P.tiles_x; tc = (t1 - t0) * P.tiles_x;
        if (r->origin_mode == RDR_ORIGIN_GRID) { r0 = t0 * TILE * r->nx; cnt = std::min<int64_t>(t1 * TILE, r->ny) * r->nx - r0; }
        else { r0 = tb * BLOCK; cnt = std::min<int64_t>((tb + tc) * BLOCK, r->n) - r0; }
    };
    int status = RDR_OK;
    auto cleanup = [&]() { for (auto& e : ev) if (e) (void)hipEventDestroy(e); };
    for (auto& e : ev)
        if (hipEventCreateWithFlags(&e, hipEventDisableTiming) != hipSuccess) { cleanup(); return fail(c, RDR_ERR_HIP, "pipelined ray tracing: event creation failed"); }
    for (int k = 0; k < nchunk && status == RDR_OK; ++k) {
        int64_t tb, tc, r0, cnt; range(k, tb, tc, r0, cnt);
        if ((d_los && hipMemcpyAsync(d_los + 3 * r0, r->los + 3 * r0, (size_t)cnt * 24, hipMemcpyHostToDevice, c->copy_stream) != hipSuccess) ||
            (d_hts && hipMemcpyAsync(d_hts + r0, r->hts + r0, (size_t)cnt * 8, hipMemcpyHostToDevice, c->copy_stream) != hipSuccess) ||
            ((d_los || d_hts) && (hipEventRecord(ev[k], c->copy_stream) != hipSuccess || hipStreamWaitEvent(c->stream, ev[k], 0) != hipSuccess))) {
            status = fail(c, RDR_ERR_HIP, "pipelined ray tracing: look-vector / height upload failed"); break;
        }
        RayParams Pk = P; Pk.ws = ws + tb * BLOCK;
        status = launch_crossings(c, q, Pk, tb, tc, nslots_total, k == 0);
    }
    for (int k = 0; k < nchunk && status == RDR_OK; ++k) {
        int64_t tb, tc, r0, cnt; range(k, tb, tc, r0, cnt);
        RayParams Pk = P; Pk.ws = ws + tb * BLOCK;
        status = launch_march(c, q, Pk, tb, tc, nslots_total);
        if (status == RDR_OK && hipEventRecord(ev[nchunk + k], c->stream) != hipSuccess) status = fail(c, RDR_ERR_HIP, "pipelined ray tracing: event");
    }
    for (int k = 0; k < nchunk && status == RDR_OK; ++k) {
        int64_t tb, tc, r0, cnt; range(k, tb, tc, r0, cnt);
        if (hipStreamWaitEvent(c->copy_stream, ev[nchunk + k], 0) != hipSuccess ||
            hipMemcpyAsync(wet + r0, dw + r0, (size_t)cnt * 8, hipMemcpyDeviceToHost, c->copy_stream) != hipSuccess ||
            hipMemcpyAsync(hydro + r0, dh + r0, (size_t)cnt * 8, hipMemcpyDeviceToHost, c->copy_stream) != hipSuccess)
            status = fail(c, RDR_ERR_HIP, "pipelined ray tracing: output download failed");
    }
    if (hipStreamSynchronize(c->copy_stream) != hipSuccess && status == RDR_OK) status = fail(c, RDR_ERR_HIP, "pipelined ray tracing: sync");
    if (hipStreamSynchronize(c->stream) != hipSuccess && status == RDR_OK) status = fail(c, RDR_ERR_HIP, "pipelined ray tracing: sync");
    cleanup();
    return status;
}

static int flags_to_status(rdr_ctx* c, int flags) {
    if (!(flags & RDR_FLAG_ANY_FINITE)) return fail(c, RDR_ERR_ALL_NAN, "geo2rdr did not converge. Check orbit coverage");
    if (flags & RDR_FLAG_ANY_NAN) return fail(c, RDR_ERR_NAN_LENGTH, "some ray lengths are NaN: the number of integration parts (delay.py:283) is undefined");
    if (flags & RDR_FLAG_BAD_HEIGHT) return fail(c, RDR_ERR_INVALID, "per-ray heights: a ray starts below the height the batch's level table was built for (pass ht <= min(rays->hts))");
    if (flags & RDR_FLAG_DIVERGED) return fail(c, RDR_ERR_INVALID, "ray lengths diverged: a model level asks for fewer than 2 or more than 65536 integration parts (are the look vectors unit vectors?)");
    return RDR_OK;
}

int rdr_ray_prepass(rdr_ctx* c, const rdr_cube* q, const rdr_rays* r, double ht, double zref, double* maxlen, int32_t* flags) {
    if (!c || !q || !maxlen) return fail(c, RDR_ERR_INVALID, "rdr_ray_prepass: NULL argument");
    note_use(c, q);
    int rc = check_rays(c, r); if (rc) return rc;
    std::vector<double> lo, hi; std::vector<int> kz;
    const int K = levels_host(q->zs, ht, zref, lo, hi, kz);
    if (K == 0) return fail(c, RDR_ERR_NO_LEVELS, "no weather-model interval contributes to the ray integral (build_ray -> None)");
    HIPCHECK(c, hipSetDevice(c->device));
    RayParams P;
    rc = stage_rays(c, r, P); if (rc) return rc;
    P.ht = ht; P.zref = zref; P.max_seg = 1000.0;
    HIPCHECK(c, hipMemsetAsync(c->d_maxlen, 0, MAX_LEVELS * sizeof(unsigned long long), c->stream));
    HIPCHECK(c, hipMemsetAsync(c->d_flags, 0, sizeof(int), c->stream));
    c->wsig.valid = false;
    if (r->n > 0) {
        const bool keep = r->loc == RDR_DEVICE && P.ntiles <= ws_chunk_tiles(c, K);
        if (keep) { rc = ws_reserve(c, P.ntiles, K, P); if (rc) return rc; }
        rc = launch_crossings(c, q, P, 0, P.ntiles); if (rc) return rc;
        if (keep) wsig_set(c, q, r, ht, zref, K, true);
    }
    int f = 0, nslow[2] = {0, 0};
    HIPCHECK(c, hipMemcpyAsync(maxlen, c->d_maxlen, (size_t)K * 8, hipMemcpyDeviceToHost, c->stream));
    HIPCHECK(c, hipMemcpyAsync(&f, c->d_flags, sizeof(int), hipMemcpyDeviceToHost, c->stream));
    HIPCHECK(c, hipMemcpyAsync(nslow, c->d_nslow, 2 * sizeof(int), hipMemcpyDeviceToHost, c->stream));
    HIPCHECK(c, hipStreamSynchronize(c->stream));
    c->last_nslow = nslow[0]; c->last_nskip = nslow[1];
    if (flags) *flags = f;
    return RDR_OK;
}

int rdr_ray_prepass_device(rdr_ctx* c, const rdr_cube* q, const rdr_rays* r, double ht, double zref, double* partition) {
    if (!c || !q || !partition) return fail(c, RDR_ERR_INVALID, "rdr_ray_prepass_device: NULL argument");
    note_use(c, q);
    int rc = check_rays(c, r); if (rc) return rc;
    if (r->loc != RDR_DEVICE) return fail(c, RDR_ERR_INVALID, "rdr_ray_prepass_device: rays must be device arrays");
    std::vector<double> lo, hi; std::vector<int> kz;
    const int K = levels_host(q->zs, ht, zref, lo, hi, kz);
    if (K == 0) return fail(c, RDR_ERR_NO_LEVELS, "no weather-model interval contributes to the ray integral (build_ray -> None)");
    HIPCHECK(c, hipSetDevice(c->device));
    RayParams P;
    rc = stage_rays(c, r, P); if (rc) return rc;
    P.ht = ht; P.zref = zref; P.max_seg = 1000.0;
    HIPCHECK(c, hipMemsetAsync(c->d_maxlen, 0, MAX_LEVELS * sizeof(unsigned long long), c->stream));
    HIPCHECK(c, hipMemsetAsync(c->d_flags, 0, sizeof(int), c->stream));
    c->wsig.valid = false;
    if (r->n > 0) {
        const bool keep = P.ntiles <= ws_chunk_tiles(c, K);
        if (keep) { rc = ws_reserve(c, P.ntiles, K, P); if (rc) return rc; }
        rc = launch_crossings(c, q, P, 0, P.ntiles); if (rc) return rc;
        if (keep) wsig_set(c, q, r, ht, zref, K, true);
    }
    hipLaunchKernelGGL(pack_partition_kernel, dim3(1), dim3(256), 0, c->stream, c->d_maxlen, c->d_flags, K, partition);
    HIPCHECK(c, hipGetLastError());
    return RDR_OK;
}

int rdr_ray_march_device(rdr_ctx* c, const rdr_cube* q, const rdr_rays* r, double ht, double zref, double max_seg, const double* partition,
                         double* wet, double* hydro) {
    if (!c || !q || !partition || !wet || !hydro) return fail(c, RDR_ERR_INVALID, "rdr_ray_march_device: NULL argument");
    note_use(c, q);
    if (!(max_seg > 0)) return fail(c, RDR_ERR_INVALID, "rdr_ray_march_device: MAX_SEGMENT_LENGTH must be positive");
    int rc = check_rays(c, r); if (rc) return rc;
    if (r->loc != RDR_DEVICE) return fail(c, RDR_ERR_INVALID, "rdr_ray_march_device: rays and outputs must be device arrays");
    std::vector<double> lo, hi; std::vector<int> kz;
    const int K = levels_host(q->zs, ht, zref, lo, hi, kz);
    if (K == 0) return fail(c, RDR_ERR_NO_LEVELS, "no weather-model interval contributes to the ray integral (build_ray -> None)");
    if (r->n == 0) return RDR_OK;
    HIPCHECK(c, hipSetDevice(c->device));
    const bool reuse = wsig_match(c, q, r, ht, zref, K);
    RayParams P;
    rc = stage_rays(c, r, P); if (rc) return rc;
    P.ht = ht; P.zref = zref; P.max_seg = max_seg;
    P.wet = wet; P.hyd = hydro;
    hipLaunchKernelGGL(unpack_partition_kernel, dim3(1), dim3(256), 0, c->stream, partition, K, c->d_maxlen, c->d_flags);
    HIPCHECK(c, hipGetLastError());
    if (reuse) { ws_attach(c, P); rc = launch_march(c, q, P, 0, P.ntiles); }
    else rc = ray_passes(c, q, P, K, P.ntiles, 1, ws_chunk_tiles(c, K), 1, false);
    c->wsig.valid = false;
    return rc;
}

int rdr_ray_march(rdr_ctx* c, const rdr_cube* q, const rdr_rays* r, double ht, double zref, const int32_t* nparts, int32_t flags,
                  double* wet, double* hydro) {
    if (!c || !q || !nparts || !wet || !hydro) return fail(c, RDR_ERR_INVALID, "rdr_ray_march: NULL argument");
    note_use(c, q);
    int rc = check_rays(c, r); if (rc) return rc;
    std::vector<double> lo, hi; std::vector<int> kz;
    const int K = levels_host(q->zs, ht, zref, lo, hi, kz);
    if (K == 0) return fail(c, RDR_ERR_NO_LEVELS, "no weather-model interval contributes to the ray integral (build_ray -> None)");
    for (int k = 0; k < K; ++k) if (nparts[k] < 2 || nparts[k] > MAX_NPARTS) return fail(c, RDR_ERR_INVALID, "rdr_ray_march: nparts out of range (2..65536)");
    if (r->n == 0) return RDR_OK;
    HIPCHECK(c, hipSetDevice(c->device));
    const bool reuse = wsig_match(c, q, r, ht, zref, K);
    RayParams P;
    rc = stage_rays(c, r, P); if (rc) return rc;
    P.ht = ht; P.zref = zref; P.max_seg = 1000.0;
    HIPCHECK(c, hipMemcpyAsync(c->d_nparts, nparts, (size_t)K * sizeof(int), hipMemcpyHostToDevice, c->stream));
    int f = flags;
    HIPCHECK(c, hipMemcpyAsync(c->d_flags, &f, sizeof(int), hipMemcpyHostToDevice, c->stream));
    HIPCHECK(c, hipStreamSynchronize(c->stream));
    P.nparts_override = c->d_nparts;
    void *dw, *dh;
    rc = stage_out(c, SLOT_OUT0, wet, (size_t)r->n * 8, r->loc, &dw); if (rc) return rc;
    rc = stage_out(c, SLOT_OUT1, hydro, (size_t)r->n * 8, r->loc, &dh); if (rc) return rc;
    P.wet = (double*)dw; P.hyd = (double*)dh;
    if (reuse) { ws_attach(c, P); rc = launch_march(c, q, P, 0, P.ntiles); }
    else rc = ray_passes(c, q, P, K, P.ntiles, 1, ws_chunk_tiles(c, K), 1, false);
    c->wsig.valid = false;
    if (rc) return rc;
    rc = finish_out(c, wet, dw, (size_t)r->n * 8, r->loc); if (rc) return rc;
    rc = finish_out(c, hydro, dh, (size_t)r->n * 8, r->loc); if (rc) return rc;
    if (r->loc == RDR_HOST) HIPCHECK(c, hipStreamSynchronize(c->stream));
    return RDR_OK;
}

static int raytrace_impl(rdr_ctx* c, const char* who, const rdr_cube* const* qs, int32_t D, const rdr_rays* r, double ht, double zref,
                         double max_seg, double* wet, double* hydro, int32_t* nparts_out, int32_t* flags_out) {
    const rdr_cube* q = qs[0];
    for (int32_t e = 0; e < D; ++e) note_use(c, qs[e]);
    if (!(max_seg > 0)) return fail(c, RDR_ERR_INVALID, std::string(who) + ": MAX_SEGMENT_LENGTH must be positive");
    int rc = check_rays(c, r); if (rc) return rc;
    std::vector<double> lo, hi; std::vector<int> kz;
    const int K = levels_host(q->zs, ht, zref, lo, hi, kz);
    if (K == 0) return fail(c, RDR_ERR_NO_LEVELS, "no weather-model interval contributes to the ray integral (build_ray -> None)");
    if (r->n == 0) return RDR_OK;
    HIPCHECK(c, hipSetDevice(c->device));
    RayParams P;
    bool pipelined = D == 1 && r->loc == RDR_HOST && r->n >= (1 << 21) && pipelining();
    const bool los_chunks = pipelined && r->los_mode == RDR_LOS_VEC;
    const bool hts_chunks = pipelined && r->hts != nullptr;
    rdr_rays rr = *r;
    if (los_chunks) rr.los = nullptr;
    if (hts_chunks) rr.hts = nullptr;
    rc = stage_rays(c, &rr, P); if (rc) return rc;
    if (pipelined && P.ntiles > ws_chunk_tiles(c, K)) {
        const void* d;
        if (los_chunks) {
            rc = stage_in(c, SLOT_IN3, r->los, (size_t)r->n * 24, r->loc, &d); if (rc) return rc;
            P.los = (const double*)d;
        }
        if (hts_chunks) {
            rc = stage_in(c, SLOT_IN6, r->hts, (size_t)r->n * 8, r->loc, &d); if (rc) return rc;
            P.ht_ray = (const double*)d;
        }
        pipelined = false;
    }
    P.ht = ht; P.zref = zref; P.max_seg = max_seg;
    const size_t bytes = (size_t)r->n * (size_t)D * 8;
    void *dw, *dh;
    rc = stage_out(c, SLOT_OUT0, wet, bytes, r->loc, &dw); if (rc) return rc;
    rc = stage_out(c, SLOT_OUT1, hydro, bytes, r->loc, &dh); if (rc) return rc;
    P.wet = (double*)dw; P.hyd = (double*)dh;
    HIPCHECK(c, hipMemsetAsync(c->d_maxlen, 0, MAX_LEVELS * sizeof(unsigned long long), c->stream));
    HIPCHECK(c, hipMemsetAsync(c->d_flags, 0, sizeof(int), c->stream));
    c->wsig.valid = false;
    if (pipelined) {
        void *dl = nullptr, *dhts = nullptr;
        if (los_chunks) { rc = ensure(c, SLOT_IN3, (size_t)r->n * 24, &dl); if (rc) return rc; }
        if (hts_chunks) { rc = ensure(c, SLOT_IN6, (size_t)r->n * 8, &dhts); if (rc) return rc; }
        rc = raytrace_pipelined(c, q, r, P, K, (double*)dl, (double*)dhts, (double*)dw, (double*)dh, wet, hydro); if (rc) return rc;
    } else {
        std::function<int(const RayParams&, int64_t, int64_t)> march;
        if (D > 1) march = [&](const RayParams& Pm, int64_t tb, int64_t tc) { return launch_march_epochs(c, qs, D, Pm, tb, tc, (int64_t)r->n); };
        rc = ray_passes(c, q, P, K, P.ntiles, 1, ws_chunk_tiles(c, K), 1, true, march); if (rc) return rc;
        rc = finish_out(c, wet, dw, bytes, r->loc); if (rc) return rc;
        rc = finish_out(c, hydro, dh, bytes, r->loc); if (rc) return rc;
    }
    const bool need_sync = r->loc == RDR_HOST || nparts_out || flags_out;
    if (need_sync) {
        std::vector<double> ml(K);
        int f = 0, nslow = 0;
        HIPCHECK(c, hipMemcpyAsync(ml.data(), c->d_maxlen, (size_t)K * 8, hipMemcpyDeviceToHost, c->stream));
        HIPCHECK(c, hipMemcpyAsync(&f, c->d_flags, sizeof(int), hipMemcpyDeviceToHost, c->stream));
        HIPCHECK(c, hipMemcpyAsync(&nslow, c->d_nslow, sizeof(int), hipMemcpyDeviceToHost, c->stream));
        HIPCHECK(c, hipStreamSynchronize(c->stream));
        c->last_nslow = nslow;
        if (nparts_out) rdr_nparts(ml.data(), K, max_seg, nparts_out);
        if (flags_out) *flags_out = f;
        return flags_to_status(c, f);
    }
    return RDR_OK;
}

int rdr_raytrace(rdr_ctx* c, const rdr_cube* q, const rdr_rays* r, double ht, double zref, double max_seg, double* wet,
                 double* hydro, int32_t* nparts_out, int32_t* flags_out) {
    if (!c || !q || !wet || !hydro) return fail(c, RDR_ERR_INVALID, "rdr_raytrace: NULL argument");
    return raytrace_impl(c, "rdr_raytrace", &q, 1, r, ht, zref, max_seg, wet, hydro, nparts_out, flags_out);
}

// ... 1136 lines not shown
```

### raider_amd/csrc/raider_kernels.h

```cpp
#pragma once
#include <hip/hip_runtime.h>
#include <stdint.h>
#include <type_traits>

#include "geodesy.h"
#include "geodesy_fast.h"

namespace rdr {

constexpr int TILE = 16;
constexpr int BLOCK = TILE * TILE;
constexpr int MAX_LEVELS = 512;
constexpr int MAX_NPARTS = 65536;

template <typename T2>
struct CubeView {
    const T2* v;
    const double* axes;
    int ny, nx, nz;
    double y_lo, y_hi, x_lo, x_hi, z_lo, z_hi;
    double inv_dy, inv_dx, inv_dz;
    int uni_y, uni_x, uni_z;
    int exact_y, exact_x;
    int small;
// ... 249 lines not shown
    for (int it = 0; it < iters; ++it) {
        const double hgt = ecef_height(px, py, pz);
        const double step = (h - hgt) / factor;
        px = px + lx * step; py = py + ly * step; pz = pz + lz * step;
    }
}

__device__ __forceinline__ double toa_newton_t(double ox, double oy, double oz, double lx, double ly, double lz,
                                               double h, int iters, double inv_factor) {
    double t = h;
#pragma unroll 1
    for (int it = 0; it < iters; ++it) {
        const double hgt = ecef_height(fma(t, lx, ox), fma(t, ly, oy), fma(t, lz, oz));
        t = fma(h - hgt, inv_factor, t);
    }
    return t;
}

__device__ __forceinline__ double level_top_u(const double* hpoly, double hi, double su, double ou, double gain) {
    double u = fma(hi, su, ou);
#pragma unroll
    for (int it = 0; it < 3; ++it) u = fma(hi - poly5(hpoly, u), gain, u);
    return u;
}

template <int N>
__device__ __forceinline__ void level_top_u_n(const double* hpoly, const double* hi, double su, double ou, double gain, double* u) {
#pragma unroll
    for (int j = 0; j < N; ++j) u[j] = fma(hi[j], su, ou);
#pragma unroll
    for (int it = 0; it < 3; ++it) {
        double p[N];
#pragma unroll
        for (int j = 0; j < N; ++j) p[j] = hpoly[PN - 1];
#pragma unroll
        for (int n = PN - 2; n >= 0; --n) {
#pragma unroll
            for (int j = 0; j < N; ++j) p[j] = fma(p[j], u[j], hpoly[n]);
        }
#pragma unroll
        for (int j = 0; j < N; ++j) u[j] = fma(hi[j] - p[j], gain, u[j]);
    }
}

constexpr int PX = 8;
__device__ const double XPOLY_NODES[PX] = {0.98078528040323044913, 0.83146961230254523708, 0.55557023301960222474, 0.19509032201612826785,
                                           -0.19509032201612826785, -0.55557023301960222474, -0.83146961230254523708, -0.98078528040323044913};
__device__ const double XPOLY_VINV[PX][PX] = {
    {-0.024864045922457250864, -0.025351161379823003334, 0.76980164952545230204, 0.78488295543032986324, -3.1779876260079822119, -3.2402480843731826008, 3.0614674589207181738, 3.1214451522580522856},
    {0.083522329739912365, 0.10045145186799834205, -2.5519026177451504679, -3.0691471822744071686, 9.6723408277623460247, 11.632825402935940496, -7.391036260090294049, -8.8891237283136355959},
    {-0.1870757203331861272, -0.33672740045197043705, 5.3803297424913405655, 9.6843376817517615307, -12.500767952508536122, -22.500787856406753567, 7.391036260090294049, 13.303513796840723793},
    {0.62841743651573101306, 3.2211615113525685678, -3.5982287742716423996, -18.443912220177554698, 6.0064147507541723095, 30.787866300500633524, -3.0614674589207181738, -15.692564486451687186},
    {0.62841743651573101306, -3.2211615113525685678, -3.5982287742716423996, 18.443912220177554698, 6.0064147507541723095, -30.787866300500633524, -3.0614674589207181738, 15.692564486451687186},
    {-0.1870757203331861272, 0.33672740045197043705, 5.3803297424913405655, -9.6843376817517615307, -12.500767952508536122, 22.500787856406753567, 7.391036260090294049, -13.303513796840723793},
    {0.083522329739912365, -0.10045145186799834205, -2.5519026177451504679, 3.0691471822744071686, 9.6723408277623460247, -11.632825402935940496, -7.391036260090294049, 8.8891237283136355959},
    {-0.024864045922457250864, 0.025351161379823003334, 0.76980164952545230204, -0.78488295543032986324, -3.1779876260079822119, 3.2402480843731826008, 3.0614674589207181738, -3.1214451522580522856}};

__device__ __forceinline__ double poly7(const double* c, double v) {
    double r = fma(c[7], v, c[6]);
    r = fma(r, v, c[5]);
    r = fma(r, v, c[4]);
    r = fma(r, v, c[3]);
    r = fma(r, v, c[2]);
    r = fma(r, v, c[1]);
    return fma(r, v, c[0]);
}

__device__ __forceinline__ void fit_crossing_poly(const double* hpoly, double su, double ou, double gain, double hm, double hh, double* xc) {
#pragma unroll
    for (int n = 0; n < PX; ++n) xc[n] = 0.0;
#pragma unroll 1
    for (int j = 0; j < PX; j += 2) {
        double hn[2], un[2];
        hn[0] = fma(hh, XPOLY_NODES[j], hm); hn[1] = fma(hh, XPOLY_NODES[j + 1], hm);
        level_top_u_n<2>(hpoly, hn, su, ou, gain, un);
#pragma unroll
        for (int n = 0; n < PX; ++n) xc[n] = fma(XPOLY_VINV[j + 1][n], un[1], fma(XPOLY_VINV[j][n], un[0], xc[n]));
    }
}

constexpr int WS_POLY_H = 0, WS_POLY_LAT = 6, WS_POLY_LON = 12, WS_XPOLY = 18, WS_SCALE = 26, WS_U0 = 27, WS_U1 = 28, WS_NFIELDS = 29;
constexpr int WS_ORIGIN = 0, WS_LOS = 3, WS_LAT0 = 6, WS_LON0 = 7, WS_S0 = 8, WS_C0 = 9, WS_SL0 = 10, WS_CL0 = 11, WS_SIDE = 12;

struct RayParams {
    int64_t n;
    int origin_mode, los_mode;
    int64_t nx, ny;
    const double* xpts; const double* ypts;
    const double* lat; const double* lon; const double* xyz;
    const double* los; const double* inc; const double* hd;
    double inc0, hd0;
    int nslices; int64_t tiles_per_slice;
    const double* hts;
    const double* ht_ray;
    int64_t los_stride;
    double ht, zref, max_seg;
    unsigned long long* maxlen_bits;
    int* flags;
    const int* nparts_override;
    int* nslow;
    int* tile_ctr;
    double* ws; int64_t nslots;
    double* side; int64_t side_cap;
    int* side_ctr;
    int64_t tile_begin, tile_count;
    double* wet; double* hyd;
    int64_t ntiles; int tiles_x;
    int stage_f64;
    int skip_levels;
};

__device__ inline int build_levels(const double2* ez, int nz, double ht, double zref, double* s_lo, double* s_hi, int* s_kz) {
    int K = 0;
    const double ztop = ez[nz - 1].x;
    for (int zz = 0; zz < nz - 1; ++zz) {
        double lo = ez[zz].x, hi = ez[zz + 1].x;
        if (hi == ztop) hi -= 0.01;
        if (hi < ht || lo >= zref) continue;
        if (lo < ht) lo = ht;
        if (hi > zref) hi = zref;
        if (fabs(hi - lo) < 1.0) continue;
        if (K < MAX_LEVELS) { s_lo[K] = lo; s_hi[K] = hi; s_kz[K] = zz; }
        ++K;
    }
    return min(K, MAX_LEVELS);
}

__device__ __forceinline__ int first_level(const double2* ez, int nz, const double* s_lo, const double* s_hi, const int* s_kz, int K,
                                           double hti, double& lo_i) {
    const double ztop = ez[nz - 1].x;
    int a = 0, b = K;
    while (a < b) {
        const int mid = (a + b) >> 1;
        double hr = ez[s_kz[mid] + 1].x;
        if (hr == ztop) hr -= 0.01;
        if (hr < hti) a = mid + 1; else b = mid;
    }
    for (int k = a; k < K; ++k) {
        const double lo = fmax(s_lo[k], hti);
        if (fabs(s_hi[k] - lo) < 1.0) continue;
        lo_i = lo;
        return k;
    }
    lo_i = 0.0;
    return K;
}

struct __attribute__((aligned(16))) LevelRec {
    double xv, hs;
    double step, zmid;
    double r0, r1;
    double gk, rk;
    int npkz, pad[3];
};
static_assert(sizeof(LevelRec) == 80, "LevelRec is read with fixed LDS offsets");

struct RaySmem {
    AxisTabs ax;
    double2* tab2;
    double* lo; double* hi;
    unsigned long long* mxcol;
    LevelRec* lev;
    double* step;
    double* hs;
    double* trig;
    double* xv;
    double* xmap;
    int* kz; int* np; int* K;
};
constexpr int MXCOLS = 16;
static_assert(sizeof(LevelRec) <= 8 * MXCOLS, "LevelRec aliases a level's mxcol columns");
__host__ __device__ inline int64_t table_nodes(int64_t ny, int64_t nx, int64_t nz, int exact_y, int exact_x) {
    return (exact_y ? 0 : ny) + (exact_x ? 0 : nx) + nz;
}
__device__ __forceinline__ RaySmem carve_smem(unsigned char* raw, int ny, int nx, int nz, int exact_y, int exact_x) {
    RaySmem m;
    const int nyt = exact_y ? 0 : ny, nxt = exact_x ? 0 : nx;
    m.tab2 = reinterpret_cast<double2*>(raw);
    m.ax.ey = exact_y ? nullptr : m.tab2;
    m.ax.ex = exact_x ? nullptr : m.tab2 + nyt;
    m.ax.ez = m.tab2 + nyt + nxt;
    m.lo = reinterpret_cast<double*>(m.tab2 + nyt + nxt + nz);
    m.hi = m.lo + nz;
    m.mxcol = reinterpret_cast<unsigned long long*>(m.hi + nz);
    m.lev = reinterpret_cast<LevelRec*>(m.mxcol);
    m.step = reinterpret_cast<double*>(m.mxcol + (size_t)nz * MXCOLS);
    m.hs = m.step + nz;
    m.trig = m.hs + nz;
    m.xv = m.trig + 112;
    m.xmap = m.xv + nz;
    m.kz = reinterpret_cast<int*>(m.xmap + 2);
    m.np = m.kz + nz;
    m.K = m.np + nz;
    return m;
}

inline size_t ray_smem_bytes(int64_t ny, int64_t nx, int64_t nz, int exact_y, int exact_x) {
    return (size_t)table_nodes(ny, nx, nz, exact_y, exact_x) * 16
           + (size_t)nz * 8 * 2
           + (size_t)nz * 8 * MXCOLS
           + (size_t)nz * 8 * 2 + 112 * 8
           + (size_t)nz * 8 + 16
           + (size_t)nz * 4 * 2 + 16;
}

__device__ __forceinline__ double* skip_dabs(const RaySmem& m) { return reinterpret_cast<double*>(m.K + 4); }
__device__ __forceinline__ unsigned long long* skip_floor(const RaySmem& m, int nz) { return reinterpret_cast<unsigned long long*>(m.K + 4) + 7 * nz; }
inline size_t skip_smem_bytes(int64_t nz) { return (size_t)nz * 8 * 8; }


template <typename T2>
__device__ __forceinline__ void fill_axes(const CubeView<T2>& c, const RaySmem& m) {
    const int tid = threadIdx.x;
    auto fill = [&](double2* dst, const double* g, int n) {
        for (int i = tid; i < n; i += BLOCK) {
            double2 e; e.x = g[i]; e.y = (i == n - 1) ? 0.0 : 1.0 / (g[i + 1] - g[i]);
            dst[i] = e;
        }
    };
    if (m.ax.ey) fill(const_cast<double2*>(m.ax.ey), c.axes, c.ny);
    if (m.ax.ex) fill(const_cast<double2*>(m.ax.ex), c.axes + c.ny, c.nx);
    fill(const_cast<double2*>(m.ax.ez), c.axes + c.ny + c.nx, c.nz);
    __syncthreads();
}

__device__ __forceinline__ int fill_levels(int nz, const RaySmem& m, double ht, double zref) {
    int tid = threadIdx.x;
    asm volatile("" : "+v"(tid));
    __syncthreads();
    if (tid == 0) {
        const int K = build_levels(m.ax.ez, nz, ht, zref, m.lo, m.hi, m.kz);
        *m.K = K;
        const double a = K > 1 ? m.hi[1] : (K > 0 ? m.hi[0] : 0.0), b = K > 1 ? m.hi[K - 1] : a;
        m.xmap[0] = 0.5 * (a + b);
        m.xmap[1] = fmax(0.5 * (b - a), 1.0);
    }
    __syncthreads();
    const int K = *m.K;
    const double hm = m.xmap[0], ihh = 1.0 / m.xmap[1];
    for (int k = tid; k < K; k += BLOCK) m.xv[k] = (m.hi[k] - hm) * ihh;
    __syncthreads();
    return K;
}

struct TileWalk {
    int64_t chunk; int xcd; int* ctr; int* slot;
    __device__ __forceinline__ TileWalk(int64_t count, int* counters, int* lds_slot) {
        xcd = blockIdx.x & 7; chunk = (count + 7) / 8; ctr = counters + xcd; slot = lds_slot;
    }
    __device__ __forceinline__ bool next(int64_t count, int64_t& local) {
        __syncthreads();
        if (threadIdx.x == 0) *slot = atomicAdd(ctr, 1);
        __syncthreads();
        const int64_t tt = *slot;
        local = (int64_t)xcd * chunk + tt;
        return tt < chunk && local < count;
    }
};

template <bool LCC>
__device__ __forceinline__ void tile_trig(double v, int lane, const LccParams& proj, double* trig) {
    double sv, cv;
    sincos(v * DEG_TO_RAD, &sv, &cv);
    trig[2 * lane] = sv; trig[2 * lane + 1] = cv;
    if (LCC) {
        if (lane < 16) trig[64 + lane] = lcc_rho(proj, sv, cv);
        else { double st, ct; lcc_theta(proj, v, st, ct); trig[80 + 2 * (lane - 16)] = st; trig[81 + 2 * (lane - 16)] = ct; }
    }
// ... 285 lines not shown
                double xm[PX];
#pragma unroll
                for (int n = 0; n < PX; ++n) xm[n] = xc[n] * mscale;
                double s_hi = u_hi * mscale;
                int k = 1;
                if constexpr (PR) {
                    const double s_first = s_hi;
                    for (; k < K; ++k) {
                        const double st = poly7(xm, m.xv[k]);
                        const double L = st - (k == k0 + 1 ? s_first : s_hi);
                        s_hi = st;
                        atomicMax(&mxc[k * MXCOLS], (unsigned long long)__double_as_longlong(k > k0 ? fmax(fabs(L), 0.0) : 0.0));
                    }
                }
                bool skip = false;
                if constexpr (SKIPPABLE) {
                    if (K > 2 && K <= 128 && skip_on()) {
                        const double* const dabs = skip_dabs(m);
                        const unsigned long long* const flr = skip_floor(m, c.nz);
                        double S = fabs(xm[0]);
#pragma unroll
                        for (int n = 1; n < PX; ++n) S += fabs(xm[n]);
                        if (!cnt) S = 0.0;
                        const bool finite = !__any(!(S < __builtin_inf()));
                        const float a0 = wave_max_nonneg(finite ? float_above_abs(S) : 0.0f);
                        if (finite && a0 == 0.0f) skip = true;
                        else if (finite) {
                            const int lane = tl & 63;
                            const int ka = min(lane, K - 1), kb = min(lane + 64, K - 1);
                            double Ba = 0.0, Bb = 0.0;
#pragma unroll
                            for (int n = 1; n < PX; ++n) {
                                const double an = (double)wave_max_nonneg(cnt ? float_above_abs(xm[n]) : 0.0f);
                                Ba = fma(an, dabs[(n - 1) * c.nz + ka], Ba);
                                if (K > 64) Bb = fma(an, dabs[(n - 1) * c.nz + kb], Bb);
                            }
                            const double margin = fma((double)a0, 0x1p-44, 0x1p-120);
                            Ba = fma(Ba, 1.0 + 0x1p-30, margin);
                            Bb = fma(Bb, 1.0 + 0x1p-30, margin);
                            bool ok = lane < 2 || lane >= K || (unsigned long long)__double_as_longlong(Ba) <= flr[ka];
                            if (K > 64) ok = ok && (lane + 64 >= K || (unsigned long long)__double_as_longlong(Bb) <= flr[kb]);
                            skip = !__any(!ok);
                            if (skip && lane == 0) atomicAdd(m.K + 3, 1);
                        }
                    }
                }
                if (skip) {
                    const double L = poly7(xm, m.xv[1]) - s_hi;
                    atomicMax(&mxc[MXCOLS], (unsigned long long)__double_as_longlong(fmax(fabs(L), 0.0)));
                    k = K;
                }
                for (; k + 2 <= K; k += 2) {
                    const double v0 = m.xv[k], v1 = m.xv[k + 1];
                    const double sa = poly7(xm, v0), sb = poly7(xm, v1);
                    const double La = sa - s_hi, Lb = sb - sa;
                    s_hi = sb;
                    atomicMax(&mxc[k * MXCOLS], (unsigned long long)__double_as_longlong(fmax(fabs(La), 0.0)));
                    atomicMax(&mxc[(k + 1) * MXCOLS], (unsigned long long)__double_as_longlong(fmax(fabs(Lb), 0.0)));
                }
                for (; k < K; ++k) {
                    const double st = poly7(xm, m.xv[k]);
                    const double L = st - s_hi;
                    s_hi = st;
                    atomicMax(&mxc[k * MXCOLS], (unsigned long long)__double_as_longlong(fmax(fabs(L), 0.0)));
                }
                if (PR ? (k0 + 1 < K) : (K > 1)) last_len = u_end * scale;
                if (K > 0 && cnt && !(poly5(q.h, u_end) > c.z_hi)) my_flags |= 8;
            }
            if (reduce && cnt && K > 0) my_flags |= (last_len != last_len) ? 1 : 2;
        }
    }
    flush();
    if (skip_on()) {
        __syncthreads();
        if (threadIdx.x == 0 && m.K[3] > 0) atomicAdd(P.nslow + 1, m.K[3]);
    }
}

struct SlicePartition {
    double poison;
    bool clamp_lo, clamp_hi;
};

template <bool REC>
__device__ __forceinline__ SlicePartition fill_partition(const RayParams& P, const RaySmem& m, int nz, int sl, int K) {
    int tz = threadIdx.x;
    asm volatile("" : "+v"(tz));
    if (tz == 0) m.K[1] = 0;
    __syncthreads();
    for (int k = tz; k < K; k += BLOCK) {
        int np;
        if (P.nparts_override) np = P.nparts_override[(int64_t)sl * MAX_LEVELS + k];
        else {
            const double parts = ceil(__longlong_as_double((long long)P.maxlen_bits[(int64_t)sl * MAX_LEVELS + k]) / P.max_seg) + 1.0;
            np = (parts >= 1.0 && parts <= (double)MAX_NPARTS) ? (int)parts : -1;
        }
        if (np < 2 || np > MAX_NPARTS) {
            np = 2;
            atomicOr(P.flags + sl, 16);
            m.K[1] = 1;
        }
        m.np[k] = np;
        m.step[k] = 1.0 / ((double)np - 1.0);
        m.hs[k] = 0.5e-6 * m.step[k];
        if constexpr (REC) {
            const int kzk = m.kz[k], last = nz - 1;
            const int zb = max(window2_base(nz, kzk), 0);
            LevelRec r;
            r.xv = m.xv[k]; r.hs = m.hs[k]; r.step = m.step[k];
            r.zmid = m.ax.ez[min(zb + 1, last)].x; r.r0 = m.ax.ez[zb].y; r.r1 = m.ax.ez[min(zb + 1, last)].y;
            r.gk = m.ax.ez[kzk].x; r.rk = m.ax.ez[kzk].y;
            r.npkz = np | (kzk << 17); r.pad[0] = r.pad[1] = r.pad[2] = 0;
            m.lev[k] = r;
            if (k == K - 1) { r.hs = 0.0; r.npkz = 2 | (kzk << 17); m.lev[K] = r; }
        }
    }
    __syncthreads();
    const int flags_in = P.flags[sl];
    SlicePartition s;
    s.poison = (m.K[1] || (flags_in & (1 | 32))) ? qnan() : 0.0;
    s.clamp_lo = !(flags_in & 4);
    s.clamp_hi = !(flags_in & 8);
    return s;
}

__device__ __forceinline__ void tile_ray(const RayParams& P, int64_t t, int tl, int64_t& i, bool& active) {
    if (P.origin_mode == 0) {
        const int64_t ty = t / P.tiles_x, tx = t - ty * P.tiles_x;
        const int64_t row = ty * TILE + (tl >> 4), col = tx * TILE + (tl & 15);
        active = row < P.ny && col < P.nx;
        i = row * P.nx + col;
    } else {
        i = t * BLOCK + tl;
        active = i < P.n;
    }
}

__device__ __forceinline__ void load_ray_record(const double* w, int64_t ns, RayPoly& q, double (&xc)[PX]) {
#pragma unroll
    for (int n = 0; n < PN; ++n) {
        q.h[n] = w[(int64_t)(WS_POLY_H + n) * ns];
        q.lat[n] = w[(int64_t)(WS_POLY_LAT + n) * ns];
        q.lon[n] = w[(int64_t)(WS_POLY_LON + n) * ns];
    }
#pragma unroll
    for (int n = 0; n < PX; ++n) xc[n] = w[(int64_t)(WS_XPOLY + n) * ns];
}

__device__ __forceinline__ bool lane_nocheck(double u0r, double u1r, bool active, bool mine, RayPoly& q, double (&xc)[PX], int ny, int nx) {
    if (!active) {
#pragma unroll
        for (int n = 0; n < PN; ++n) { q.lat[n] = 0.0; q.lon[n] = 0.0; }
        q.lat[0] = 0.5; q.lon[0] = 0.5;
#pragma unroll
        for (int n = 0; n < PX; ++n) xc[n] = 0.0;
        u0r = 0.0; u1r = 0.0;
    }
    auto inside = [&](const double* cf, int n) {
        const double r = 1.006 * (fabs(cf[1]) + fabs(cf[2]) + fabs(cf[3]) + fabs(cf[4]) + fabs(cf[5]));
        return (cf[0] - r >= 0.0) & (cf[0] + r < (double)(n - 1));
    };
    double xs = 0.0;
#pragma unroll
    for (int n = 0; n < PX; ++n) xs += fabs(xc[n]);
    return (mine || !active) && (fabs(u0r) <= 1.001) && (fabs(u1r) <= 1.001) && (xs <= 1.001) && inside(q.lat, ny) && inside(q.lon, nx);
}


template <typename T2, int E, bool NC>
__device__ __forceinline__ void issue_top(const CubeView<T2>& c, const EpochCubes<T2, E>& ev, const RaySmem& m, const RayPoly& q, double us, int zbase,
                                          bool floor_it, bool ceil_it, PendingSample<T2, E>& s) {
    double ph = poly5(q.h, us);
    const double plat = poly5(q.lat, us), plon = poly5(q.lon, us);
    if (floor_it) { asm volatile("" ::: "memory"); ph = fmax(ph, c.z_lo); }
    if (ceil_it) { asm volatile("" ::: "memory"); ph = fmin(ph, c.z_hi); }
    sample_issue<T2, 1, NC, E>(c, ev, m.ax, plat, plon, ph, zbase, s);
}

template <typename T2, int E, int e = 0>
__device__ __forceinline__ void finish_into(const PendingSample<T2, E>& s, double wv, double* acc_w, double* acc_h) {
    double vw, vh;
    sample_finish_lerp(s, vw, vh, e);
    acc_w[e] = fma(wv, vw, acc_w[e]); acc_h[e] = fma(wv, vh, acc_h[e]);
    if constexpr (e + 1 < E) finish_into<T2, E, e + 1>(s, wv, acc_w, acc_h);
}

template <typename T2, int E, bool NC>
__device__ __forceinline__ void march_slice_levels(const CubeView<T2>& c, const EpochCubes<T2, E>& ev, const RaySmem& m, const RayPoly& q, const double (&xc)[PX],
                                                   double u0, double u1, int K, bool clamp_lo, bool clamp_hi, unsigned long long live,
                                                   double* acc_w, double* acc_h) {
    typedef __attribute__((address_space(3))) const LevelRec LdsRec;
    int la = (int)(size_t)m.lev;
    asm volatile("" : "+v"(la));
    const LdsRec* rec = (const LdsRec*)(size_t)(unsigned)la;
    int npkz = __builtin_amdgcn_readfirstlane(rec->npkz);
    int np = npkz & 0x1ffff, kz = npkz >> 17;
    double hs = rec->hs;
    double u_k = u0;
    double u_last = u1;
    double du = u_last - u_k;
    if (K > 0) {
        PendingSample<T2, E> s;
        issue_top<T2, E, NC>(c, ev, m, q, fma(0.0 * rec->step, du, u_k), window2_base(c.nz, kz - ((m.lo[0] <= m.ax.ez[kz].x) ? 1 : 0)), clamp_lo, false, s);
        finish_into(s, hs * fabs(du), acc_w, acc_h);
    }
#pragma unroll 1
    for (int k = 0; k < K; ++k) {
        const int zbase = window2_base(c.nz, kz);
        const bool more = k + 1 < K;
        const double w_mid = (2.0 * hs) * fabs(du);
        if (np > 2) {
            const double step = rec->step, gk = rec->gk, rk = rec->rk;
#pragma unroll 1
            for (int j = 1; j < np - 1; ++j) {
                PendingSample<T2, E> s;
                const double us = fma((double)j * step, du, u_k);
                const double ph = poly5(q.h, us), plat = poly5(q.lat, us), plon = poly5(q.lon, us);
                int iz = kz;
                s.tz = (ph - gk) * rk;
                if (!(s.tz >= 0.0) || !(s.tz <= 1.0)) cell_exact(m.ax.ez, c.nz, ph, iz, s.tz);
                gather_corners<T2, E, true, NC>(c, ev, m.ax, plat, plon, iz, s);
                finish_into(s, w_mid, acc_w, acc_h);
            }
        }
        PendingSample<T2, E> top;
        {
            const double us = u_k + du;
            double ph = poly5(q.h, us);
            const double plat = poly5(q.lat, us), plon = poly5(q.lon, us);
            if (clamp_hi && !more) { asm volatile("" ::: "memory"); ph = fmin(ph, c.z_hi); }
            const double d = ph - rec->zmid;
            int iz; bool ok;
            if (__builtin_expect((__builtin_amdgcn_ballot_w64(!(d >= 0.0)) & live) == 0ULL, 1)) {
                iz = zbase + 1;
                top.tz = d * rec->r1;
                ok = top.tz <= 1.0;
            } else {
                double ds = d;
                asm volatile("" : "+v"(ds));
                const bool up = ds >= 0.0;
                iz = zbase + (int)up;
                top.tz = fma(ds, up ? rec->r1 : rec->r0, up ? 0.0 : 1.0);
                ok = (top.tz >= 0.0) & (top.tz <= 1.0);
            }
            if (!(ok & (c.nz >= 4))) cell_exact(m.ax.ez, c.nz, ph, iz, top.tz);
            gather_corners<T2, E, true, NC>(c, ev, m.ax, plat, plon, iz, top);
        }
        const double t2 = poly7(xc, rec[1].xv);
        const double du1 = t2 - u_last, hs1 = rec[1].hs;
        u_last = t2;
        const double w_top = fma(hs1, fabs(du1), hs * fabs(du));
        npkz = __builtin_amdgcn_readfirstlane(rec[1].npkz);
        finish_into(top, w_top, acc_w, acc_h);
        u_k += du; du = du1; hs = hs1;
        np = npkz & 0x1ffff; kz = npkz >> 17;
        ++rec;
    }
}

template <typename T2, int E, bool NC>
__device__ __forceinline__ void march_ray_height_levels(const CubeView<T2>& c, const EpochCubes<T2, E>& ev, const RaySmem& m, const RayPoly& q, const double (&xc)[PX],
                                                        double u0, double u1, const int& K, int k0, double lo_first, bool clamp_lo, bool clamp_hi,
                                                        double* acc_w, double* acc_h) {
    int kmin = k0;
#pragma unroll
    for (int off = 32; off > 0; off >>= 1) kmin = min(kmin, __shfl_xor(kmin, off, 64));
    kmin = __builtin_amdgcn_readfirstlane(kmin);
    const bool has = k0 < K;
    const int kf = has ? k0 : 0;
    double u_k = has ? u0 : 0.0, u_last = has ? u1 : 0.0;
    double du = u_last - u_k;
    if (K > 0) {
        const int kzf = m.kz[kf];
        PendingSample<T2, E> s;
        issue_top<T2, E, NC>(c, ev, m, q, fma(0.0 * m.step[kf], du, u_k), window2_base(c.nz, kzf - ((lo_first <= m.ax.ez[kzf].x) ? 1 : 0)), clamp_lo, false, s);
        if (has) finish_into(s, m.hs[kf] * fabs(du), acc_w, acc_h);
    }
#pragma unroll 1
    for (int k = kmin; k < K; ++k) {
        const int np = __builtin_amdgcn_readfirstlane(m.np[k]);
        const int kz = __builtin_amdgcn_readfirstlane(m.kz[k]);
        const double step = m.step[k], hs = m.hs[k];
        const bool more = k + 1 < K;
        if (k >= k0) {
            const int zbase = window2_base(c.nz, kz);
            const double w_mid = (2.0 * hs) * fabs(du);
#pragma unroll 1
            for (int j = 1; j < np - 1; ++j) {
                PendingSample<T2, E> s;
                const double us = fma((double)j * step, du, u_k);
                const double ph = poly5(q.h, us);
                const double plat = poly5(q.lat, us), plon = poly5(q.lon, us);
                sample_issue<T2, 2, NC, E>(c, ev, m.ax, plat, plon, ph, kz, s);
                finish_into(s, w_mid, acc_w, acc_h);
            }
            PendingSample<T2, E> top;
            issue_top<T2, E, NC>(c, ev, m, q, u_k + du, zbase, false, clamp_hi && !more, top);
            double du1 = 0.0;
            double w_top = hs * fabs(du);
            if (more) {
                const double t2 = poly7(xc, m.xv[k + 1]);
                du1 = t2 - u_last; u_last = t2;
                w_top = fma(m.hs[k + 1], fabs(du1), w_top);
            }
            finish_into(top, w_top, acc_w, acc_h);
            u_k += du; du = du1;
        }
    }
}

template <typename T2, bool SLOW, int GRID = 0, bool PR = false>
__global__ __launch_bounds__(BLOCK) __attribute__((amdgpu_waves_per_eu(SLOW ? 1 : (sizeof(T2) == 16 ? 3 : 4), SLOW ? 8 : (sizeof(T2) == 16 ? 3 : 4)))) void march_kernel(CubeView<T2> c_in, RayParams P, LccParams proj) {
    static_assert(!SLOW || !PR, "the generic kernel looks at P.ht_ray at run time");
    if (SLOW && *P.nslow == 0) return;
    const bool per_ray = PR || (SLOW && P.ht_ray != nullptr);
    constexpr bool REGULAR = GRID == 1;
    CubeView<T2> c = c_in;
    if (REGULAR) { c.exact_y = 1; c.exact_x = 1; c.small = 1; }
    if (GRID == 2) { c.exact_y = 0; c.exact_x = 0; c.uni_y = 1; c.uni_x = 1; c.small = 1; }
    extern __shared__ __attribute__((aligned(16))) unsigned char smem_raw[];
    const RaySmem m = carve_smem(smem_raw, c.ny, c.nx, c.nz, c.exact_y, c.exact_x);
    constexpr bool STAGED = !SLOW && !PR && REGULAR && sizeof(T2) == 16;
    constexpr int STAGE_N = 48;
    __shared__ T2 s_stage[STAGED ? (BLOCK / 64) * STAGE_N : 1];
    fill_axes(c, m);
    const int tid = threadIdx.x;
    int K = 0, slice = -1;
    double poison = 0.0;
    bool clamp_lo = false, clamp_hi = false, clamp_any = false;
    TileWalk walk(P.tile_count, P.tile_ctr, m.K + 2);
    int64_t lt;
    while (walk.next(P.tile_count, lt)) {
        const int64_t tg = P.tile_begin + lt;
        const int sl = (int)(tg / P.tiles_per_slice);
        const int64_t t = tg - (int64_t)sl * P.tiles_per_slice;
        if (sl != slice) {
            slice = sl;
            K = fill_levels(c.nz, m, P.hts ? P.hts[sl] : P.ht, P.zref);
            const SlicePartition part = fill_partition<!SLOW && !PR>(P, m, c.nz, sl, K);
            poison = part.poison; clamp_lo = part.clamp_lo; clamp_hi = part.clamp_hi;
            clamp_any = clamp_lo | clamp_hi;
        }
        int tl = threadIdx.x;
        asm volatile("" : "+v"(tl));
        int64_t i; bool active;
        tile_ray(P, t, tl, i, active);
        const double* w = P.ws + (lt * BLOCK + tl);
        const int64_t ns = P.nslots;
        const double scale_rec = w[(int64_t)WS_SCALE * ns];
        const bool fast_ok = !active || scale_rec != 0.0;
        const bool mine = SLOW ? !fast_ok : fast_ok;
        if (SLOW && !__any(mine)) continue;
        double acc_w = 0.0, acc_h = 0.0;
        int k0 = 0; double lo_first = K > 0 ? m.lo[0] : 0.0;
        if (PR || SLOW) {
            if (per_ray) k0 = (active && mine) ? first_level(m.ax.ez, c.nz, m.lo, m.hi, m.kz, K, P.ht_ray[i], lo_first) : K;
        }
        if constexpr (!SLOW) {
            RayPoly q;
            double xc[PX];
            load_ray_record(w, ns, q, xc);
            const double scale = scale_rec;
            const double u0r = w[(int64_t)WS_U0 * ns], u1r = w[(int64_t)WS_U1 * ns];
            const EpochCubes<T2, 1> one{{c.v}};
            const unsigned long long live = __builtin_amdgcn_ballot_w64(active && mine);
            auto run = [&](auto nochk) {
                constexpr bool NC = decltype(nochk)::value;
                if constexpr (PR) march_ray_height_levels<T2, 1, NC>(c, one, m, q, xc, u0r, u1r, K, k0, lo_first, clamp_lo, clamp_hi, &acc_w, &acc_h);
                else march_slice_levels<T2, 1, NC>(c, one, m, q, xc, u0r, u1r, K, clamp_lo, clamp_hi, live, &acc_w, &acc_h);
            };
            bool lane_safe = false;
            if (REGULAR) lane_safe = lane_nocheck(u0r, u1r, active, mine, q, xc, c.ny, c.nx);
            auto run_staged = [&]() {
                T2* const st = s_stage + (tl >> 6) * STAGE_N;
                const int lane = tl & 63;
                unsigned lane_off = ((unsigned)((lane >> 2) & 3) * (unsigned)c.nx + (unsigned)(lane & 3)) * (unsigned)c.nz + (unsigned)(lane >> 4);
                asm volatile("" : "+v"(lane_off));
                const bool loader = lane < STAGE_N;
                bool stage_on = true;
                const char* const vb = reinterpret_cast<const char*>(c.v);
                const size_t rowx = (size_t)c.nz * sizeof(T2), rowy = (size_t)c.nx * rowx;
                int fy0 = 0, fx0 = 0, zb = 0;
                auto fetch = [&](int iy, int ix, int iz, PendingSample<T2>& sm) {
                    const unsigned ry = (unsigned)(iy - fy0), rx = (unsigned)(ix - fx0), rz = (unsigned)(iz - zb);
                    bool staged_here = false;
                    if (stage_on) {
                        const bool out = active & (max(max(ry, rx), rz + 1u) > 2u);
                        staged_here = __builtin_amdgcn_ballot_w64(out) == 0;
                        stage_on = staged_here;
                    }
                    if (staged_here) {
                        typedef decltype(T2().x) S1;
                        typedef S1 S2 __attribute__((ext_vector_type(2)));
                        typedef __attribute__((address_space(3))) S2 LdsS2;
                        const LdsS2* p = (const LdsS2*)st + (active ? (rz * 16u + ry * 4u + rx) : 0u);
                        auto get = [&](int i_, int o_) { const S2 t_ = p[o_]; sm.v[0][i_].x = t_.x; sm.v[0][i_].y = t_.y; };
                        get(0, 0); get(1, 16); get(2, 1); get(3, 17); get(4, 4); get(5, 20); get(6, 5); get(7, 21);
                        asm volatile("" ::: "memory");
                    } else {
                        const unsigned off = (__umul24(__umul24((unsigned)iy, (unsigned)c.nx) + (unsigned)ix, (unsigned)c.nz) + (unsigned)iz) * (unsigned)sizeof(T2);
                        const T2* p00 = reinterpret_cast<const T2*>(vb + off);
                        const T2* p01 = reinterpret_cast<const T2*>(vb + rowx + off);
                        const T2* p10 = reinterpret_cast<const T2*>(vb + rowy + off);
                        const T2* p11 = reinterpret_cast<const T2*>(vb + rowy + rowx + off);
                        T2* const v = sm.v[0];
                        v[0] = p00[0]; v[1] = p00[1]; v[2] = p01[0]; v[3] = p01[1];
                        v[4] = p10[0]; v[5] = p10[1]; v[6] = p11[0]; v[7] = p11[1];
                    }
                };
                auto finish = [&](const PendingSample<T2>& sm, double wv) {
                    double vw, vh;
                    sample_finish_lerp(sm, vw, vh);
                    acc_w = fma(wv, vw, acc_w); acc_h = fma(wv, vh, acc_h);
                };
                int np = __builtin_amdgcn_readfirstlane(m.np[0]);
                int kz = __builtin_amdgcn_readfirstlane(m.kz[0]);
                double step = m.step[0], hs = m.hs[0];
                double u_k = w[(int64_t)WS_U0 * ns];
                double u_last = w[(int64_t)WS_U1 * ns];
                double du = u_last - u_k;
                if (K > 0) {
                    PendingSample<T2> s0;
                    double ph = poly5(q.h, fma(0.0 * step, du, u_k));
                    const double plat = poly5(q.lat, fma(0.0 * step, du, u_k)), plon = poly5(q.lon, fma(0.0 * step, du, u_k));
                    if (clamp_lo) { asm volatile("" ::: "memory"); ph = fmax(ph, c.z_lo); }
                    sample_issue<T2, 1, true>(c, m.ax, plat, plon, ph, window2_base(c.nz, kz - ((m.lo[0] <= m.ax.ez[kz].x) ? 1 : 0)), s0);
                    finish(s0, hs * fabs(du));
                }
#pragma unroll 1
                for (int k = 0; k < K; ++k) {
                    zb = window2_base(c.nz, kz);
                    const bool more = k + 1 < K;
                    const double w_mid = (2.0 * hs) * fabs(du);
                    PendingSample<T2> top;
                    double ph = poly5(q.h, u_k + du);
                    const double plat = poly5(q.lat, u_k + du), plon = poly5(q.lon, u_k + du);
                    if (clamp_hi && !more) { asm volatile("" ::: "memory"); ph = fmin(ph, c.z_hi); }
                    int iy, ix, iz;
                    cell_xy<true, true>(m.ax.ey, c.ny, plat, c.y_lo, c.y_hi, c.inv_dy, true, true, iy, top.ty);
                    cell_xy<true, true>(m.ax.ex, c.nx, plon, c.x_lo, c.x_hi, c.inv_dx, true, true, ix, top.tx);
                    window2_cell(m.ax.ez, c.nz, ph, zb, c.nz >= 4, iz, top.tz);
                    if (stage_on) {
                        fy0 = min(max(__builtin_amdgcn_readfirstlane(iy) - 1, 0), c.ny - 4);
                        fx0 = min(max(__builtin_amdgcn_readfirstlane(ix) - 1, 0), c.nx - 4);
                        const unsigned base = (unsigned)__builtin_amdgcn_readfirstlane((fy0 * c.nx + fx0) * c.nz + zb);
                        __builtin_amdgcn_wave_barrier();
                        if (loader) st[lane] = c.v[base + lane_off];
                        __builtin_amdgcn_wave_barrier();
                    }
#pragma unroll 1
                    for (int j = 1; j < np - 1; ++j) {
                        PendingSample<T2> sm;
// ... 90 lines not shown
```

### raider_amd/engine.py

```python
import ctypes as C

import numpy as np

from . import _lib as L
from . import _pinned
from ._lib import Context, check, f64, ptr


def _is_dev(a):
    return hasattr(a, 'data_ptr')


def _dev_f64(t, what, numel=None):
    import torch
    if t.dtype != torch.float64 or not t.is_cuda or not t.is_contiguous():
        raise TypeError(f'{what} must be a contiguous float64 tensor on the GPU (got {t.dtype} on {t.device}, contiguous={t.is_contiguous()})')
    if numel is not None and t.numel() != numel:
        raise ValueError(f'{what} has {t.numel()} elements, {numel} expected')
    return t


def _dev_points(ctx, y, x, z, inc, divisor):
    if inc is not None and divisor is not None:
        raise ValueError('give inc= or divisor=, not both')
    ctx.adopt_torch_stream(y)
    if x is None:
        if y.shape[-1] != 3:
            raise ValueError(f'The requested sample points xi have dimension {y.shape[-1]} but this RegularGridInterpolator has dimension 3')
        _dev_f64(y, 'pts')
        return tuple(y.shape[:-1]), y.numel() // 3
    n = y.numel()
    for t, what in ((y, 'y'), (x, 'x'), (z, 'z')):
        _dev_f64(t, what, n)
    return tuple(y.shape), n


def _delay_outputs(rays, out, lead=()):
    if out is not None:
        return out
    shape = tuple(lead) + tuple(rays.shape)
    if rays._torch_device is not None:
        import torch
        wet = torch.empty(shape, dtype=torch.float64, device=rays._torch_device)
        return wet, torch.empty_like(wet)
    return _pinned.empty(shape), _pinned.empty(shape)


class Cube:

    def __init__(self, ys, xs, zs, wet, hydro, order='yxz', ctx=None):
        self.ctx = ctx or Context.default()
        self.handle = None
        ys, xs, zs = f64(ys), f64(xs), f64(zs)
        dev = _is_dev(wet)
        if not dev:
            wet = np.asarray(wet)
            hydro = np.asarray(hydro)
            if wet.dtype.kind != 'f' or wet.dtype.itemsize not in (4, 8):
                wet = wet.astype(np.float64)
            if hydro.dtype != wet.dtype:
                hydro = hydro.astype(wet.dtype)
            wet = np.ascontiguousarray(wet)
            hydro = np.ascontiguousarray(hydro)
            dt = L.RDR_F32 if wet.dtype.itemsize == 4 else L.RDR_F64
            if not wet.dtype.isnative:
                dt |= L.RDR_BYTESWAPPED
            shape = wet.shape
        else:
            import torch
            if wet.dtype not in (torch.float32, torch.float64) or hydro.dtype != wet.dtype:
                raise TypeError(f'device cubes must be float32 or float64 tensors of one dtype (got {wet.dtype} / {hydro.dtype})')
            if not (wet.is_cuda and hydro.is_cuda and wet.is_contiguous() and hydro.is_contiguous()):
                raise ValueError('device cubes must be contiguous tensors on the GPU')
            dt = L.RDR_F32 if wet.dtype == torch.float32 else L.RDR_F64
            shape = tuple(wet.shape)
            self.ctx.adopt_torch_stream(wet)
        ny, nx, nz = ys.size, xs.size, zs.size
        if order == 'yxz':
            want = (ny, nx, nz)
            sy, sx, sz = nx * nz, nz, 1
        elif order == 'zyx':
            want = (nz, ny, nx)
            sy, sx, sz = nx, 1, ny * nx
        else:
            raise ValueError("order must be 'yxz' or 'zyx'")
        if tuple(shape) != want or tuple(hydro.shape) != want:
            raise ValueError(f'There are {want} points in the grid but values have shape {tuple(shape)}')
        h = C.c_void_p()
        check(self.ctx.lib.rdr_cube_create(self.ctx.handle, ptr(ys), ny, ptr(xs), nx, ptr(zs), nz, ptr(wet), ptr(hydro), dt,
# ... 165 lines not shown
        if x is None:
            y = np.asarray(y)
            if y.shape[-1] != 3:
                raise ValueError(f'The requested sample points xi have dimension {y.shape[-1]} but this RegularGridInterpolator has dimension 3')
            shape = y.shape[:-1]
            ya, xa, za = f64(y).reshape(-1, 3), None, None
            n = ya.shape[0]
        else:
            y, x, z = np.broadcast_arrays(np.asarray(y), np.asarray(x), np.asarray(z))
            shape = y.shape
            ya, xa, za = f64(y).reshape(-1), f64(x).reshape(-1), f64(z).reshape(-1)
            n = ya.size
        mode, parr, inc0 = 0, None, 0.0
        if inc is not None:
            if np.ndim(inc) == 0:
                mode, inc0 = 2, float(inc)
            else:
                mode, parr = 1, f64(np.broadcast_to(np.asarray(inc, dtype=np.float64), shape)).reshape(-1)
        elif divisor is not None:
            mode, parr = 3, f64(np.broadcast_to(np.asarray(divisor, dtype=np.float64), shape)).reshape(-1)
        return ya, xa, za, n, shape, mode, parr, inc0

    def point_delays(self, xpts, ypts, zpts, y, x=None, z=None, inc=None, divisor=None, grid=None):
        gx, gy, gz = f64(xpts).ravel(), f64(ypts).ravel(), f64(np.atleast_1d(zpts)).ravel()
        ya, xa, za, n, shape, mode, parr, inc0 = self._point_args(y, x, z, inc, divisor)
        wet = _pinned.empty((n,)); hyd = _pinned.empty((n,))
        flag = C.c_int32(0)
        tail = (ptr(gx), gx.size, ptr(gy), gy.size, ptr(gz), gz.size, ptr(ya), ptr(xa), ptr(za), n, mode, ptr(parr), inc0, ptr(wet), ptr(hyd), C.byref(flag))
        if grid is None:
            check(self.ctx.lib.rdr_point_delays(self.ctx.handle, self.handle, *tail), self.ctx.handle)
        else:
            kind, gp = grid[0], f64(grid[1])
            check(self.ctx.lib.rdr_point_delays_grid(self.ctx.handle, self.handle, int(kind), ptr(gp), gp.size, *tail), self.ctx.handle)
        return wet.reshape(shape), hyd.reshape(shape), bool(flag.value)

    def build_delay_cube(self, xpts, ypts, zpts, grid=None):
        x, y, z = f64(xpts).ravel(), f64(ypts).ravel(), f64(np.atleast_1d(zpts)).ravel()
        h = C.c_void_p()
        tail = (ptr(x), x.size, ptr(y), y.size, ptr(z), z.size, L.RDR_HOST, C.byref(h))
        if grid is None:
            check(self.ctx.lib.rdr_build_cube_to_cube(self.ctx.handle, self.handle, *tail), self.ctx.handle)
        else:
            gp = f64(grid[1])
            check(self.ctx.lib.rdr_build_cube_grid_to_cube(self.ctx.handle, self.handle, int(grid[0]), ptr(gp), gp.size, *tail), self.ctx.handle)
        return Cube._from_handle(self.ctx, h)

    def build_cube(self, xpts, ypts, zpts, out=None, want_nan=False, grid=None):
        if grid is None:
            build = lambda *a: self.ctx.lib.rdr_build_cube(self.ctx.handle, self.handle, *a)
        else:
            gp = f64(grid[1])
            build = lambda *a: self.ctx.lib.rdr_build_cube_grid(self.ctx.handle, self.handle, int(grid[0]), ptr(gp), gp.size, *a)
        if _is_dev(xpts):
            import torch
            self.ctx.adopt_torch_stream(xpts)
            nx, ny, nz = xpts.numel(), ypts.numel(), zpts.numel()
            for t, what in ((xpts, 'xpts'), (ypts, 'ypts'), (zpts, 'zpts')):
                _dev_f64(t, what)
            wet, hyd = out if out is not None else (torch.empty((nz, ny, nx), dtype=torch.float64, device=xpts.device),
                                                    torch.empty((nz, ny, nx), dtype=torch.float64, device=xpts.device))
            _dev_f64(wet, 'out[0]', nx * ny * nz); _dev_f64(hyd, 'out[1]', nx * ny * nz)
            check(build(ptr(xpts), nx, ptr(ypts), ny, ptr(zpts), nz, ptr(wet), ptr(hyd), L.RDR_DEVICE), self.ctx.handle)
            return (wet, hyd, None) if want_nan else (wet, hyd)
        x, y, z = f64(xpts).ravel(), f64(ypts).ravel(), f64(np.atleast_1d(zpts)).ravel()
        wet = _pinned.empty((z.size, y.size, x.size)); hyd = _pinned.empty((z.size, y.size, x.size))
        with self.ctx.lock:
            check(build(ptr(x), x.size, ptr(y), y.size, ptr(z), z.size, ptr(wet), ptr(hyd), L.RDR_HOST), self.ctx.handle)
            f = self.ctx.lib.rdr_last_nan_output(self.ctx.handle)
        if want_nan:
            return wet, hyd, (None if f < 0 else bool(f))
        return wet, hyd

    def ray_kernel_attributes(self, which):
        v = [C.c_int32() for _ in range(5)]
        check(self.ctx.lib.rdr_ray_kernel_attributes(self.ctx.handle, self.handle, int(which), *[C.byref(x) for x in v]), self.ctx.handle)
        return dict(zip(('vgpr', 'lds_static', 'lds_dynamic', 'scratch', 'max_threads'), (x.value for x in v)))

    def ray_levels(self, ht, zref):
        nz = self.shape[2]
        K = C.c_int32()
        lo, hi, kz = np.empty(nz), np.empty(nz), np.empty(nz, dtype=np.int32)
        check(self.ctx.lib.rdr_ray_levels(self.handle, float(ht), float(zref), C.byref(K), ptr(lo), ptr(hi), ptr(kz)), self.ctx.handle)
        return lo[:K.value].copy(), hi[:K.value].copy(), kz[:K.value].copy()

    def ray_prepass(self, rays, ht, zref):
        rays.adopt_stream(self.ctx)
        ht = rays.table_height(ht)
        K = len(self.ray_levels(ht, zref)[0])
        maxlen = np.zeros(K)
        flags = C.c_int32()
        check(self.ctx.lib.rdr_ray_prepass(self.ctx.handle, self.handle, C.byref(rays.struct), float(ht), float(zref), ptr(maxlen),
                                           C.byref(flags)), self.ctx.handle)
        return maxlen, flags.value

    def _check_partition(self, partition, ht, zref):
        K = len(self.ray_levels(ht, zref)[0])
        _dev_f64(partition, 'partition')
        if partition.numel() < K + 4:
            raise ValueError(f'partition needs K + 4 = {K + 4} elements (got {partition.numel()})')

    def ray_prepass_device(self, rays, ht, zref, partition):
        rays.adopt_stream(self.ctx)
        ht = rays.table_height(ht)
        self._check_partition(partition, ht, zref)
        check(self.ctx.lib.rdr_ray_prepass_device(self.ctx.handle, self.handle, C.byref(rays.struct), float(ht), float(zref), ptr(partition)),
              self.ctx.handle)
        return partition

    def ray_march_device(self, rays, ht, zref, partition, max_seg=1000.0, out=None):
        rays.adopt_stream(self.ctx)
        ht = rays.table_height(ht)
        wet, hyd = out if out is not None else rays.empty_outputs()
        rays.check_outputs(wet, hyd)
        self._check_partition(partition, ht, zref)
        check(self.ctx.lib.rdr_ray_march_device(self.ctx.handle, self.handle, C.byref(rays.struct), float(ht), float(zref), float(max_seg),
                                                ptr(partition), ptr(wet), ptr(hyd)), self.ctx.handle)
        return wet, hyd

    def ray_march(self, rays, ht, zref, nparts, flags, out=None):
        rays.adopt_stream(self.ctx)
        ht = rays.table_height(ht)
        nparts = np.ascontiguousarray(nparts, dtype=np.int32)
        wet, hyd = out if out is not None else rays.empty_outputs()
        rays.check_outputs(wet, hyd)
        check(self.ctx.lib.rdr_ray_march(self.ctx.handle, self.handle, C.byref(rays.struct), float(ht), float(zref), ptr(nparts),
                                         int(flags), ptr(wet), ptr(hyd)), self.ctx.handle)
        return wet, hyd

    def raytrace(self, rays, ht, zref, max_seg=1000.0, out=None, want_nparts=True):
        return _trace_batch(self, self.ctx.lib.rdr_raytrace, (self.handle,), (), rays, ht, zref, max_seg, out, want_nparts)

    def raytrace_slices(self, rays, hts, zref, max_seg=1000.0, out=None, want_partition=True, want_nan=False):
        hts = _slice_heights(self.ctx, rays, hts, 'a batch with per-ray heights is ONE slice: use raytrace()')
        return _trace_slices(self.ctx, self.ctx.lib.rdr_raytrace_slices, (self.handle,), (), self.shape[2] - 1, rays, hts, zref, max_seg, out,
                             want_partition, want_nan)

    def raytrace_slices_to_cube(self, rays, hts, zref, max_seg=1000.0):
        hts = _slice_heights(self.ctx, rays, hts, 'a batch with per-ray heights is ONE slice: use raytrace()')
        (cube,), K, nparts, flags = _trace_slices_to_cubes(self.ctx, self.ctx.lib.rdr_raytrace_slices_to_cube, (self.handle,), (), self.shape[2] - 1,
                                                         rays, hts, zref, max_seg)
        return cube, K, nparts, flags

    def __del__(self):
        try:
            if getattr(self, 'handle', None):
                self.ctx.lib.rdr_cube_destroy(self.handle)
                self.handle = None
        except Exception:
            pass


def epoch_groups(D, emax=4):
    emax = 4 if emax >= 4 else (2 if emax >= 2 else 1)
    out, left = [], int(D)
    while left > 0:
        g = 4 if (left >= 4 and emax >= 4) else (2 if (left >= 2 and emax >= 2) else 1)
        out.append(g); left -= g
    return out


def _slice_heights(ctx, rays, hts, per_ray_heights):
    rays.adopt_stream(ctx)
    if rays.ht_min is not None:
        raise ValueError(per_ray_heights)
    hts = f64(np.atleast_1d(hts)).ravel()
    if rays.slices not in (0, hts.size):
# ... 404 lines not shown
```

Before: 2.763 billion rays/s.

## Precompute per-slice level records in a global table read via constant address space

Per-level records (step, half weight, z-cell ratios, packed np/kz) used to be built in LDS inside every march block. They are now built once per slice by a separate level_table_kernel into a device buffer, and the march loop reads them through scalar/constant-address loads. The next record is prefetched into registers while the current level is processed. This aims to cut redundant per-block setup and LDS traffic and to put wave-uniform data in scalar registers, at the cost of an extra kernel launch, a global buffer, and a new host API for inspecting the table.

```diff
diff --git a/include/raider_hip.h b/include/raider_hip.h
--- a/include/raider_hip.h
+++ b/include/raider_hip.h
@@ -163,6 +163,9 @@
 int rdr_ray_march_device(rdr_ctx* ctx, const rdr_cube* cube, const rdr_rays* rays, double ht, double zref, double max_seg,
                          const double* partition, double* wet, double* hydro);
 
+int rdr_level_table(rdr_ctx* ctx, const rdr_cube* cube, const double* hts, int32_t nslices, double zref, const int32_t* nparts,
+                    const double* maxlen, int32_t ld, double max_seg, void* records);
+
 int rdr_ray_march(rdr_ctx* ctx, const rdr_cube* cube, const rdr_rays* rays, double ht, double zref,
                   const int32_t* nparts, int32_t flags, double* wet, double* hydro);
 int rdr_raytrace(rdr_ctx* ctx, const rdr_cube* cube, const rdr_rays* rays, double ht, double zref,
diff --git a/raider_amd/_lib.py b/raider_amd/_lib.py
--- a/raider_amd/_lib.py
+++ b/raider_amd/_lib.py
@@ -125,6 +125,7 @@
     ('rdr_look_vectors', C.c_int, [_VP, C.POINTER(RdrRays), C.c_double, _VP]),
     ('rdr_ray_prepass_device', C.c_int, [_VP, _VP, _VP, C.c_double, C.c_double, _VP]),
     ('rdr_ray_march_device', C.c_int, [_VP, _VP, _VP, C.c_double, C.c_double, C.c_double, _VP, _VP, _VP]),
+    ('rdr_level_table', C.c_int, [_VP, _VP, _VP, C.c_int32, C.c_double, _VP, _VP, C.c_int32, C.c_double, _VP]),
     ('rdr_inverse_time_weights', C.c_int, [_VP, _VP, C.c_int64, _VP, C.c_int32, C.c_double, C.c_double, _VP, C.c_int]),
     ('rdr_cube_blend_weighted', C.c_int, [_VP, C.POINTER(_VP), C.c_int32, _VP, C.c_int, C.POINTER(_VP)]),
     ('rdr_cube_blend_azimuth_time', C.c_int, [_VP, C.POINTER(_VP), C.POINTER(_VP), C.c_int32, _VP, _VP, C.c_int, _VP, _VP, _VP, C.c_int64, _VP, C.c_double,
diff --git a/raider_amd/csrc/epoch_kernels.h b/raider_amd/csrc/epoch_kernels.h
--- a/raider_amd/csrc/epoch_kernels.h
+++ b/raider_amd/csrc/epoch_kernels.h
@@ -34,7 +34,7 @@
         if (sl != slice) {
             slice = sl;
             K = fill_levels(c.nz, m, P.hts ? P.hts[sl] : P.ht, P.zref);
-            const SlicePartition part = fill_partition<!PR>(P, m, c.nz, sl, K);
+            const SlicePartition part = fill_partition(P, m, sl, K);
             poison = part.poison; clamp_lo = part.clamp_lo; clamp_hi = part.clamp_hi;
         }
         int tl = threadIdx.x;
@@ -56,10 +56,11 @@
         const double scale = scale_rec;
         const double u0r = w[(int64_t)WS_U0 * ns], u1r = w[(int64_t)WS_U1 * ns];
         const unsigned long long live = __builtin_amdgcn_ballot_w64(active && mine);
+        const LevelRec* const lev = PR ? nullptr : P.lev + (int64_t)__builtin_amdgcn_readfirstlane(sl) * (c.nz + 1);
         auto run = [&](auto nochk) {
             constexpr bool NC = decltype(nochk)::value;
             if constexpr (PR) march_ray_height_levels<T2, E, NC>(c, ev, m, q, xc, u0r, u1r, K, k0, lo_first, clamp_lo, clamp_hi, acc_w, acc_h);
-            else march_slice_levels<T2, E, NC>(c, ev, m, q, xc, u0r, u1r, K, clamp_lo, clamp_hi, live, acc_w, acc_h);
+            else march_slice_levels<T2, E, NC>(c, ev, m, q, xc, lev, u0r, u1r, K, clamp_lo, clamp_hi, live, acc_w, acc_h);
         };
         bool lane_safe = false;
         if (REGULAR) lane_safe = lane_nocheck(u0r, u1r, active, mine, q, xc, c.ny, c.nx);
diff --git a/raider_amd/csrc/raider_hip.hip b/raider_amd/csrc/raider_hip.hip
--- a/raider_amd/csrc/raider_hip.hip
+++ b/raider_amd/csrc/raider_hip.hip
@@ -58,6 +58,7 @@
     DevBuf ws;
     DevBuf side;
     int64_t side_cap = 0;
+    DevBuf lev;
     int* d_sidectr = nullptr;
     int* h_word = nullptr;
     struct PinSlot { void* p = nullptr; size_t cap = 0; hipEvent_t ev = nullptr; bool used = false; };
@@ -368,6 +369,7 @@
     if (c->d_tilectr) (void)hipFree(c->d_tilectr);
     if (c->ws.p) (void)hipFree(c->ws.p);
     if (c->side.p) (void)hipFree(c->side.p);
+    if (c->lev.p) (void)hipFree(c->lev.p);
     if (c->d_sidectr) (void)hipFree(c->d_sidectr);
     if (c->h_word) (void)hipHostFree(c->h_word);
     if (c->nan_words) (void)hipHostFree(c->nan_words);
@@ -479,6 +481,7 @@
     if ((c->ws.p && c->ws.cap > keep) || (c->side.p && c->side.cap > keep)) c->wsig.valid = false;
     drop(c->ws);
     if (c->side.p && c->side.cap > keep) { drop(c->side); c->side_cap = 0; }
+    drop(c->lev);
     std::lock_guard<std::recursive_mutex> guard(g_view_mutex);
     while (!c->cube_pool.empty() && c->cube_pool_bytes > keep) {
         rdr_ctx::PoolEntry e = c->cube_pool.front();
@@ -1904,6 +1907,31 @@
     return (!per_ray && !q->exact[0] && !q->exact[1] && q->uni[0] && q->uni[1]) ? 2 : 0;
 }
 
+static int launch_level_table(rdr_ctx* c, const rdr_cube* q, RayParams& P, int64_t s0, int64_t ns) {
+    P.lev = nullptr;
+    if (P.ht_ray || ns <= 0) return RDR_OK;
+    const size_t need = (size_t)P.nslices * (size_t)(q->nz + 1) * sizeof(LevelRec);
+    if (c->lev.cap < need) {
+        if (c->lev.p) { HIPCHECK(c, hipStreamSynchronize(c->stream)); HIPCHECK(c, hipFree(c->lev.p)); c->lev.p = nullptr; c->lev.cap = 0; }
+        { const int rc_ = dev_malloc(c, &c->lev.p, need); if (rc_) return rc_; }
+        c->lev.cap = need;
+    }
+    P.lev = (const LevelRec*)c->lev.p;
+    hipError_t e;
+    {
+        KTimer t(c, 1);
+        e = launch_lds(level_table_kernel<float2>, dim3((unsigned)ns), dim3(BLOCK), ray_smem_bytes(0, 0, q->nz, 1, 1), c->stream, make_view<float2>(q), P, (int)s0,
+                       (LevelRec*)c->lev.p);
+    }
+    if (e != hipSuccess) return fail(c, RDR_ERR_HIP, std::string("level_table_kernel launch: ") + hipGetErrorString(e));
+    return RDR_OK;
+}
+
+static int check_level_table(rdr_ctx* c, const RayParams& P) {
+    if (!P.ht_ray && !P.lev) return fail(c, RDR_ERR_INVALID, "pass 2 was launched without its level table (launch_level_table)");
+    return RDR_OK;
+}
+
 static int launch_march_generic(rdr_ctx* c, const rdr_cube* q, RayParams P, dim3 G, dim3 B, size_t sm, bool zero_ctr) {
     if (zero_ctr) HIPCHECK(c, hipMemsetAsync(c->d_tilectr + 24, 0, 8 * sizeof(int), c->stream));
     P.tile_ctr = c->d_tilectr + 24;
@@ -1916,6 +1944,7 @@
 
 static int launch_march(rdr_ctx* c, const rdr_cube* q, RayParams P, int64_t tb, int64_t tc, int64_t nslots_total = 0) {
     P.tile_begin = tb; P.tile_count = tc; P.nslots = nslots_total > 0 ? nslots_total : tc * BLOCK;
+    { const int rc = check_level_table(c, P); if (rc) return rc; }
     static const int stage_f64 = []() { const char* e = std::getenv("RAIDER_HIP_F64_STAGE"); return e ? std::atoi(e) : 1; }();
     P.stage_f64 = stage_f64;
     const int g = ray_grid(c, tc, 8);
@@ -1958,6 +1987,7 @@
 
 static int launch_march_epochs(rdr_ctx* c, const rdr_cube* const* qs, int D, RayParams P, int64_t tb, int64_t tc, int64_t estride) {
     const rdr_cube* q = qs[0];
+    { const int rc = check_level_table(c, P); if (rc) return rc; }
     const int emax = epochs_max();
     const bool per_ray = P.ht_ray != nullptr;
     const int grid = march_grid(q, per_ray);
@@ -2029,6 +2059,7 @@
             int rc = ws_reserve(c, ns * per, K, Pg); if (rc) return rc;
             rc = launch_crossings(c, q, Pg, s0 * per, ns * per); if (rc) return rc;
             Pg.maxlen_bits = P.maxlen_bits;
+            rc = launch_level_table(c, q, Pg, s0, ns); if (rc) return rc;
             rc = pass2(Pg, s0 * per, ns * per); if (rc) return rc;
             if (after_group) { rc = after_group(s0, ns); if (rc) return rc; }
         }
@@ -2043,6 +2074,7 @@
         }
         RayParams Pw = P;
         rc = ws_reserve(c, fit, K, Pw); if (rc) return rc;
+        rc = launch_level_table(c, q, Pw, s, 1); if (rc) return rc;
         for (int64_t tb = 0; tb < per; tb += fit) {
             const int64_t tc = std::min<int64_t>(fit, per - tb);
             RayParams Pc = Pw;
@@ -2085,6 +2117,7 @@
         RayParams Pk = P; Pk.ws = ws + tb * BLOCK;
         status = launch_crossings(c, q, Pk, tb, tc, nslots_total, k == 0);
     }
+    if (status == RDR_OK) status = launch_level_table(c, q, P, 0, 1);
     for (int k = 0; k < nchunk && status == RDR_OK; ++k) {
         int64_t tb, tc, r0, cnt; range(k, tb, tc, r0, cnt);
         RayParams Pk = P; Pk.ws = ws + tb * BLOCK;
@@ -2187,10 +2220,42 @@
     P.wet = wet; P.hyd = hydro;
     hipLaunchKernelGGL(unpack_partition_kernel, dim3(1), dim3(256), 0, c->stream, partition, K, c->d_maxlen, c->d_flags);
     HIPCHECK(c, hipGetLastError());
-    if (reuse) { ws_attach(c, P); rc = launch_march(c, q, P, 0, P.ntiles); }
+    if (reuse) { ws_attach(c, P); rc = launch_level_table(c, q, P, 0, 1); if (!rc) rc = launch_march(c, q, P, 0, P.ntiles); }
     else rc = ray_passes(c, q, P, K, P.ntiles, 1, ws_chunk_tiles(c, K), 1, false);
     c->wsig.valid = false;
     return rc;
+}
+
+int rdr_level_table(rdr_ctx* c, const rdr_cube* q, const double* hts, int32_t nslices, double zref, const int32_t* nparts, const double* maxlen,
+                    int32_t ld, double max_seg, void* records) {
+    if (!c || !q || !hts || !records || (nparts == nullptr) == (maxlen == nullptr))
+        return fail(c, RDR_ERR_INVALID, "rdr_level_table: NULL argument, or not exactly one of nparts / maxlen");
+    if (nslices < 1 || nslices > MAX_SLICES) return fail(c, RDR_ERR_INVALID, "rdr_level_table: 1..512 slices per call");
+    if (ld < (int32_t)q->nz - 1 || ld > MAX_LEVELS) return fail(c, RDR_ERR_INVALID, "rdr_level_table: rows of nz-1 .. 512 entries");
+    if (maxlen && !(max_seg > 0)) return fail(c, RDR_ERR_INVALID, "rdr_level_table: MAX_SEGMENT_LENGTH must be positive");
+    note_use(c, q);
+    HIPCHECK(c, hipSetDevice(c->device));
+    RayParams P;
+    std::memset(&P, 0, sizeof(P));
+    P.nslices = nslices; P.ht = hts[0]; P.zref = zref; P.max_seg = maxlen ? max_seg : 1000.0;
+    std::vector<unsigned long long> rows(maxlen ? (size_t)nslices * MAX_LEVELS : 0, 0ULL);
+    std::vector<int> irows(nparts ? (size_t)nslices * MAX_LEVELS : 0, 0);
+    for (int s = 0; s < nslices; ++s)
+        for (int k = 0; k < ld; ++k) {
+            if (nparts) irows[(size_t)s * MAX_LEVELS + k] = nparts[(size_t)s * ld + k];
+            else std::memcpy(&rows[(size_t)s * MAX_LEVELS + k], &maxlen[(size_t)s * ld + k], 8);
+        }
+    const void *dht, *drows;
+    int rc = stage_in(c, SLOT_AUX, hts, (size_t)nslices * 8, RDR_HOST, &dht); if (rc) return rc;
+    rc = nparts ? stage_in(c, SLOT_IN4, irows.data(), irows.size() * sizeof(int), RDR_HOST, &drows)
+                : stage_in(c, SLOT_IN4, rows.data(), rows.size() * 8, RDR_HOST, &drows);
+    if (rc) return rc;
+    P.hts = (const double*)dht;
+    if (nparts) P.nparts_override = (const int*)drows; else P.maxlen_bits = (unsigned long long*)const_cast<void*>(drows);
+    rc = launch_level_table(c, q, P, 0, nslices); if (rc) return rc;
+    HIPCHECK(c, hipMemcpyAsync(records, P.lev, (size_t)nslices * (size_t)(q->nz + 1) * sizeof(LevelRec), hipMemcpyDeviceToHost, c->stream));
+    HIPCHECK(c, hipStreamSynchronize(c->stream));
+    return RDR_OK;
 }
 
 int rdr_ray_march(rdr_ctx* c, const rdr_cube* q, const rdr_rays* r, double ht, double zref, const int32_t* nparts, int32_t flags,
@@ -2217,7 +2282,7 @@
     rc = stage_out(c, SLOT_OUT0, wet, (size_t)r->n * 8, r->loc, &dw); if (rc) return rc;
     rc = stage_out(c, SLOT_OUT1, hydro, (size_t)r->n * 8, r->loc, &dh); if (rc) return rc;
     P.wet = (double*)dw; P.hyd = (double*)dh;
-    if (reuse) { ws_attach(c, P); rc = launch_march(c, q, P, 0, P.ntiles); }
+    if (reuse) { ws_attach(c, P); rc = launch_level_table(c, q, P, 0, 1); if (!rc) rc = launch_march(c, q, P, 0, P.ntiles); }
     else rc = ray_passes(c, q, P, K, P.ntiles, 1, ws_chunk_tiles(c, K), 1, false);
     c->wsig.valid = false;
     if (rc) return rc;
diff --git a/raider_amd/csrc/raider_kernels.h b/raider_amd/csrc/raider_kernels.h
--- a/raider_amd/csrc/raider_kernels.h
+++ b/raider_amd/csrc/raider_kernels.h
@@ -355,6 +355,7 @@
 constexpr int WS_POLY_H = 0, WS_POLY_LAT = 6, WS_POLY_LON = 12, WS_XPOLY = 18, WS_SCALE = 26, WS_U0 = 27, WS_U1 = 28, WS_NFIELDS = 29;
 constexpr int WS_ORIGIN = 0, WS_LOS = 3, WS_LAT0 = 6, WS_LON0 = 7, WS_S0 = 8, WS_C0 = 9, WS_SL0 = 10, WS_CL0 = 11, WS_SIDE = 12;
 
+struct LevelRec;
 struct RayParams {
     int64_t n;
     int origin_mode, los_mode;
@@ -377,6 +378,7 @@
     double* side; int64_t side_cap;
     int* side_ctr;
     int64_t tile_begin, tile_count;
+    const LevelRec* lev;
     double* wet; double* hyd;
     int64_t ntiles; int tiles_x;
     int stage_f64;
@@ -426,14 +428,13 @@
     double gk, rk;
     int npkz, pad[3];
 };
-static_assert(sizeof(LevelRec) == 80, "LevelRec is read with fixed LDS offsets");
+static_assert(sizeof(LevelRec) == 80, "LevelRec is the host-visible record of rdr_level_table (include/raider_hip.h)");
 
 struct RaySmem {
     AxisTabs ax;
     double2* tab2;
     double* lo; double* hi;
     unsigned long long* mxcol;
-    LevelRec* lev;
     double* step;
     double* hs;
     double* trig;
@@ -442,7 +443,6 @@
     int* kz; int* np; int* K;
 };
 constexpr int MXCOLS = 16;
-static_assert(sizeof(LevelRec) <= 8 * MXCOLS, "LevelRec aliases a level's mxcol columns");
 __host__ __device__ inline int64_t table_nodes(int64_t ny, int64_t nx, int64_t nz, int exact_y, int exact_x) {
     return (exact_y ? 0 : ny) + (exact_x ? 0 : nx) + nz;
 }
@@ -456,7 +456,6 @@
     m.lo = reinterpret_cast<double*>(m.tab2 + nyt + nxt + nz);
     m.hi = m.lo + nz;
     m.mxcol = reinterpret_cast<unsigned long long*>(m.hi + nz);
-    m.lev = reinterpret_cast<LevelRec*>(m.mxcol);
     m.step = reinterpret_cast<double*>(m.mxcol + (size_t)nz * MXCOLS);
     m.hs = m.step + nz;
     m.trig = m.hs + nz;
@@ -908,38 +907,34 @@
     bool clamp_lo, clamp_hi;
 };
 
-template <bool REC>
-__device__ __forceinline__ SlicePartition fill_partition(const RayParams& P, const RaySmem& m, int nz, int sl, int K) {
+__device__ __forceinline__ int level_nparts(const RayParams& P, int sl, int k, bool& diverged) {
+    int np;
+    if (P.nparts_override) np = P.nparts_override[(int64_t)sl * MAX_LEVELS + k];
+    else {
+        const double parts = ceil(__longlong_as_double((long long)P.maxlen_bits[(int64_t)sl * MAX_LEVELS + k]) / P.max_seg) + 1.0;
+        np = (parts >= 1.0 && parts <= (double)MAX_NPARTS) ? (int)parts : -1;
+    }
+    diverged = np < 2 || np > MAX_NPARTS;
+    return diverged ? 2 : np;
+}
+__device__ __forceinline__ double level_step(int np) { return 1.0 / ((double)np - 1.0); }
+__device__ __forceinline__ double level_half_weight(double step) { return 0.5e-6 * step; }
+
+__device__ __forceinline__ SlicePartition fill_partition(const RayParams& P, const RaySmem& m, int sl, int K) {
     int tz = threadIdx.x;
     asm volatile("" : "+v"(tz));
     if (tz == 0) m.K[1] = 0;
     __syncthreads();
     for (int k = tz; k < K; k += BLOCK) {
-        int np;
-        if (P.nparts_override) np = P.nparts_override[(int64_t)sl * MAX_LEVELS + k];
-        else {
-            const double parts = ceil(__longlong_as_double((long long)P.maxlen_bits[(int64_t)sl * MAX_LEVELS + k]) / P.max_seg) + 1.0;
-            np = (parts >= 1.0 && parts <= (double)MAX_NPARTS) ? (int)parts : -1;
-        }
-        if (np < 2 || np > MAX_NPARTS) {
-            np = 2;
+        bool diverged;
+        const int np = level_nparts(P, sl, k, diverged);
+        if (diverged) {
             atomicOr(P.flags + sl, 16);
             m.K[1] = 1;
         }
         m.np[k] = np;
-        m.step[k] = 1.0 / ((double)np - 1.0);
-        m.hs[k] = 0.5e-6 * m.step[k];
-        if constexpr (REC) {
-            const int kzk = m.kz[k], last = nz - 1;
-            const int zb = max(window2_base(nz, kzk), 0);
-            LevelRec r;
-            r.xv = m.xv[k]; r.hs = m.hs[k]; r.step = m.step[k];
-            r.zmid = m.ax.ez[min(zb + 1, last)].x; r.r0 = m.ax.ez[zb].y; r.r1 = m.ax.ez[min(zb + 1, last)].y;
-            r.gk = m.ax.ez[kzk].x; r.rk = m.ax.ez[kzk].y;
-            r.npkz = np | (kzk << 17); r.pad[0] = r.pad[1] = r.pad[2] = 0;
-            m.lev[k] = r;
-            if (k == K - 1) { r.hs = 0.0; r.npkz = 2 | (kzk << 17); m.lev[K] = r; }
-        }
+        m.step[k] = level_step(np);
+        m.hs[k] = level_half_weight(m.step[k]);
     }
     __syncthreads();
     const int flags_in = P.flags[sl];
@@ -948,6 +943,43 @@
     s.clamp_lo = !(flags_in & 4);
     s.clamp_hi = !(flags_in & 8);
     return s;
+}
+
+__device__ __forceinline__ LevelRec make_level_rec(const RaySmem& m, int nz, int k, int np) {
+    const int kzk = m.kz[k], last = nz - 1;
+    const int zb = max(window2_base(nz, kzk), 0);
+    LevelRec r;
+    r.step = level_step(np); r.hs = level_half_weight(r.step); r.xv = m.xv[k];
+    r.zmid = m.ax.ez[min(zb + 1, last)].x; r.r0 = m.ax.ez[zb].y; r.r1 = m.ax.ez[min(zb + 1, last)].y;
+    r.gk = m.ax.ez[kzk].x; r.rk = m.ax.ez[kzk].y;
+    r.npkz = np | (kzk << 17); r.pad[0] = r.pad[1] = r.pad[2] = 0;
+    return r;
+}
+
+template <typename T2>
+__global__ __launch_bounds__(BLOCK) void level_table_kernel(CubeView<T2> c, RayParams P, int first_slice, LevelRec* table) {
+    c.exact_y = 1; c.exact_x = 1;
+    extern __shared__ __attribute__((aligned(16))) unsigned char smem_raw[];
+    const RaySmem m = carve_smem(smem_raw, c.ny, c.nx, c.nz, 1, 1);
+    fill_axes(c, m);
+    const int sl = first_slice + (int)blockIdx.x;
+    const int K = fill_levels(c.nz, m, P.hts ? P.hts[sl] : P.ht, P.zref);
+    LevelRec* const out = table + (int64_t)sl * (c.nz + 1);
+    for (int k = threadIdx.x; k <= c.nz; k += BLOCK) {
+        LevelRec r;
+        if (k < K) {
+            bool diverged;
+            r = make_level_rec(m, c.nz, k, level_nparts(P, sl, k, diverged));
+        } else if (k == K && K > 0) {
+            bool diverged;
+            r = make_level_rec(m, c.nz, K - 1, level_nparts(P, sl, K - 1, diverged));
+            r.hs = 0.0; r.npkz = 2 | (m.kz[K - 1] << 17);
+        } else {
+            r.xv = r.hs = r.step = r.zmid = r.r0 = r.r1 = r.gk = r.rk = 0.0;
+            r.npkz = 0; r.pad[0] = r.pad[1] = r.pad[2] = 0;
+        }
+        out[k] = r;
+    }
 }
 
 __device__ __forceinline__ void tile_ray(const RayParams& P, int64_t t, int tl, int64_t& i, bool& active) {
@@ -1011,32 +1043,38 @@
     if constexpr (e + 1 < E) finish_into<T2, E, e + 1>(s, wv, acc_w, acc_h);
 }
 
+struct LevelRegs { double xv, hs, step, zmid, r0, r1, gk, rk; int npkz; };
+typedef __attribute__((address_space(4))) const LevelRec ConstLevelRec;
+__device__ __forceinline__ LevelRegs load_level(const ConstLevelRec* r) {
+    LevelRegs v;
+    v.xv = r->xv; v.hs = r->hs; v.step = r->step; v.zmid = r->zmid; v.r0 = r->r0; v.r1 = r->r1; v.gk = r->gk; v.rk = r->rk; v.npkz = r->npkz;
+    return v;
+}
+
 template <typename T2, int E, bool NC>
 __device__ __forceinline__ void march_slice_levels(const CubeView<T2>& c, const EpochCubes<T2, E>& ev, const RaySmem& m, const RayPoly& q, const double (&xc)[PX],
-                                                   double u0, double u1, int K, bool clamp_lo, bool clamp_hi, unsigned long long live,
+                                                   const LevelRec* lev, double u0, double u1, int K, bool clamp_lo, bool clamp_hi, unsigned long long live,
                                                    double* acc_w, double* acc_h) {
-    typedef __attribute__((address_space(3))) const LevelRec LdsRec;
-    int la = (int)(size_t)m.lev;
-    asm volatile("" : "+v"(la));
-    const LdsRec* rec = (const LdsRec*)(size_t)(unsigned)la;
-    int npkz = __builtin_amdgcn_readfirstlane(rec->npkz);
-    int np = npkz & 0x1ffff, kz = npkz >> 17;
-    double hs = rec->hs;
+    const ConstLevelRec* rec = (const ConstLevelRec*)(size_t)lev;
+    LevelRegs cur = load_level(rec);
+    int np = cur.npkz & 0x1ffff, kz = cur.npkz >> 17;
+    double hs = cur.hs;
     double u_k = u0;
     double u_last = u1;
     double du = u_last - u_k;
     if (K > 0) {
         PendingSample<T2, E> s;
-        issue_top<T2, E, NC>(c, ev, m, q, fma(0.0 * rec->step, du, u_k), window2_base(c.nz, kz - ((m.lo[0] <= m.ax.ez[kz].x) ? 1 : 0)), clamp_lo, false, s);
+        issue_top<T2, E, NC>(c, ev, m, q, fma(0.0 * cur.step, du, u_k), window2_base(c.nz, kz - ((m.lo[0] <= m.ax.ez[kz].x) ? 1 : 0)), clamp_lo, false, s);
         finish_into(s, hs * fabs(du), acc_w, acc_h);
     }
 #pragma unroll 1
     for (int k = 0; k < K; ++k) {
+        const LevelRegs nxt = load_level(rec + k + 1);
         const int zbase = window2_base(c.nz, kz);
         const bool more = k + 1 < K;
         const double w_mid = (2.0 * hs) * fabs(du);
         if (np > 2) {
-            const double step = rec->step, gk = rec->gk, rk = rec->rk;
+            const double step = cur.step, gk = cur.gk, rk = cur.rk;
 #pragma unroll 1
             for (int j = 1; j < np - 1; ++j) {
                 PendingSample<T2, E> s;
@@ -1055,32 +1093,31 @@
             double ph = poly5(q.h, us);
             const double plat = poly5(q.lat, us), plon = poly5(q.lon, us);
             if (clamp_hi && !more) { asm volatile("" ::: "memory"); ph = fmin(ph, c.z_hi); }
-            const double d = ph - rec->zmid;
+            const double d = ph - cur.zmid;
             int iz; bool ok;
             if (__builtin_expect((__builtin_amdgcn_ballot_w64(!(d >= 0.0)) & live) == 0ULL, 1)) {
                 iz = zbase + 1;
-                top.tz = d * rec->r1;
+                top.tz = d * cur.r1;
                 ok = top.tz <= 1.0;
             } else {
                 double ds = d;
                 asm volatile("" : "+v"(ds));
                 const bool up = ds >= 0.0;
                 iz = zbase + (int)up;
-                top.tz = fma(ds, up ? rec->r1 : rec->r0, up ? 0.0 : 1.0);
+                top.tz = fma(ds, up ? cur.r1 : cur.r0, up ? 0.0 : 1.0);
                 ok = (top.tz >= 0.0) & (top.tz <= 1.0);
             }
             if (!(ok & (c.nz >= 4))) cell_exact(m.ax.ez, c.nz, ph, iz, top.tz);
             gather_corners<T2, E, true, NC>(c, ev, m.ax, plat, plon, iz, top);
         }
-        const double t2 = poly7(xc, rec[1].xv);
-        const double du1 = t2 - u_last, hs1 = rec[1].hs;
+        const double t2 = poly7(xc, nxt.xv);
+        const double du1 = t2 - u_last, hs1 = nxt.hs;
         u_last = t2;
         const double w_top = fma(hs1, fabs(du1), hs * fabs(du));
-        npkz = __builtin_amdgcn_readfirstlane(rec[1].npkz);
         finish_into(top, w_top, acc_w, acc_h);
         u_k += du; du = du1; hs = hs1;
-        np = npkz & 0x1ffff; kz = npkz >> 17;
-        ++rec;
+        np = nxt.npkz & 0x1ffff; kz = nxt.npkz >> 17;
+        cur = nxt;
     }
 }
 
@@ -1163,7 +1200,7 @@
         if (sl != slice) {
             slice = sl;
             K = fill_levels(c.nz, m, P.hts ? P.hts[sl] : P.ht, P.zref);
-            const SlicePartition part = fill_partition<!SLOW && !PR>(P, m, c.nz, sl, K);
+            const SlicePartition part = fill_partition(P, m, sl, K);
             poison = part.poison; clamp_lo = part.clamp_lo; clamp_hi = part.clamp_hi;
             clamp_any = clamp_lo | clamp_hi;
         }
@@ -1190,10 +1227,11 @@
             const double u0r = w[(int64_t)WS_U0 * ns], u1r = w[(int64_t)WS_U1 * ns];
             const EpochCubes<T2, 1> one{{c.v}};
             const unsigned long long live = __builtin_amdgcn_ballot_w64(active && mine);
+            const LevelRec* const lev = PR ? nullptr : P.lev + (int64_t)__builtin_amdgcn_readfirstlane(sl) * (c.nz + 1);
             auto run = [&](auto nochk) {
                 constexpr bool NC = decltype(nochk)::value;
                 if constexpr (PR) march_ray_height_levels<T2, 1, NC>(c, one, m, q, xc, u0r, u1r, K, k0, lo_first, clamp_lo, clamp_hi, &acc_w, &acc_h);
-                else march_slice_levels<T2, 1, NC>(c, one, m, q, xc, u0r, u1r, K, clamp_lo, clamp_hi, live, &acc_w, &acc_h);
+                else march_slice_levels<T2, 1, NC>(c, one, m, q, xc, lev, u0r, u1r, K, clamp_lo, clamp_hi, live, &acc_w, &acc_h);
             };
             bool lane_safe = false;
             if (REGULAR) lane_safe = lane_nocheck(u0r, u1r, active, mine, q, xc, c.ny, c.nx);
diff --git a/raider_amd/engine.py b/raider_amd/engine.py
--- a/raider_amd/engine.py
+++ b/raider_amd/engine.py
@@ -5,6 +5,10 @@
 from . import _lib as L
 from . import _pinned
 from ._lib import Context, check, f64, ptr
+
+
+LEVEL_REC = np.dtype([('xv', '<f8'), ('hs', '<f8'), ('step', '<f8'), ('zmid', '<f8'), ('r0', '<f8'), ('r1', '<f8'), ('gk', '<f8'), ('rk', '<f8'),
+                      ('npkz', '<i4'), ('pad', '<i4', (3,))])
 
 
 def _is_dev(a):
@@ -336,6 +340,22 @@
         lo, hi, kz = np.empty(nz), np.empty(nz), np.empty(nz, dtype=np.int32)
         check(self.ctx.lib.rdr_ray_levels(self.handle, float(ht), float(zref), C.byref(K), ptr(lo), ptr(hi), ptr(kz)), self.ctx.handle)
         return lo[:K.value].copy(), hi[:K.value].copy(), kz[:K.value].copy()
+
+    def level_table(self, hts, zref, nparts=None, maxlen=None, max_seg=1000.0):
+        hts = f64(np.atleast_1d(hts)).ravel()
+        nz = self.shape[2]
+        if (nparts is None) == (maxlen is None):
+            raise ValueError('exactly one of nparts / maxlen')
+        if nparts is not None:
+            rows = np.ascontiguousarray(np.atleast_2d(nparts), dtype=np.int32)
+        else:
+            rows = np.ascontiguousarray(np.atleast_2d(maxlen), dtype=np.float64)
+        if rows.shape[0] != hts.size:
+            raise ValueError(f'{hts.size} slices, {rows.shape[0]} partition rows')
+        out = np.zeros((hts.size, nz + 1), dtype=LEVEL_REC)
+        check(self.ctx.lib.rdr_level_table(self.ctx.handle, self.handle, ptr(hts), hts.size, float(zref), ptr(rows) if nparts is not None else None,
+                                           None if nparts is not None else ptr(rows), rows.shape[1], float(max_seg), ptr(out)), self.ctx.handle)
+        return out
 
     def ray_prepass(self, rays, ht, zref):
         rays.adopt_stream(self.ctx)
```

Result: faster. 2.848 billion rays/s, median of 6 (+3.1%).
